# claforte/RayTracingWeekend.jl

Measured on AMD Instinct MI355X. Metric: Msamples/s (pixels x spp) on scene_random_spheres 1920x1080, higher is better.
Workload: dtype f32

## Files before the change

raytracingweekend.jl_amd/csrc/rtw_kernels.hpp:

```cpp
#pragma once
#include "rtw_device.hpp"

namespace rtw {

#define RTW_JOB_PX 16
#ifndef RTW_SLOT_BYTES
#define RTW_SLOT_BYTES 4608
#endif
#define RTW_REF_BITS 9
#define RTW_REF_MASK 511u
#define RTW_SLOT_FREE 0xffffffffu
#define RTW_SLOT_OPENING 0xfffffffeu
#define RTW_SLOT_OPENING_BIT 0x80000000u
#define RTW_JOB_EOF 0xffffffffu
#define RTW_JOB_RETRY 0xfffffffeu

struct KParams {
    int width, height, spp, max_depth;
    uint64_t seed;
    int n_chunks;
    int chunk_spp;
    int shard_index, shard_count;
    int tiles_i, tiles_j;
    unsigned total_jobs;
    unsigned local_tiles;
    unsigned bpj;
    unsigned n_slots, slot_stride;
    unsigned job_shift;
    unsigned rows_shift;
    unsigned div_bpj_m, div_bpj_s, div_tiles_m, div_tiles_s;
    int gamma;
    int out_layout;
    int drain_profile;
};

struct DevCounters {
    unsigned next_job[8];
    unsigned long long segments;
    unsigned long long samples;
    unsigned long long phase[32];
    unsigned long long t_first, t_last, t_end_sum, n_waves;
    unsigned end_hist[4096];
};

struct JobSlot {
    unsigned ready_seq;
    unsigned job;
    int remaining;
    unsigned valid;
    int i_base, j_base;
    unsigned k_tile;
    unsigned pad;
    double uv[12];
    __device__ __forceinline__ unsigned long long *acc(unsigned px) { return reinterpret_cast<unsigned long long *>(this + 1) + 8u * px; }
    __device__ __forceinline__ const unsigned long long *acc(unsigned px) const { return reinterpret_cast<const unsigned long long *>(this + 1) + 8u * px; }
};
static_assert(sizeof(JobSlot) == 128, "JobSlot header is 128 bytes (16-byte aligned accumulators follow)");
template <typename T> struct BatchArgs {
    const Camera<T> *cams;
    const unsigned long long *seeds;
    unsigned tiles_jv;
    unsigned div_tjv_m, div_tjv_s;
    unsigned long long view_elems;
};
struct AccumArgs {
    unsigned long long *words;
    int chunk_begin;
    int samples;
};
struct JobCache { unsigned long long jc; unsigned jc_lock; unsigned queue_off; unsigned last_g; unsigned static_used; };
template <typename T> struct WgShared {
    unsigned char slots[RTW_SLOT_BYTES];
    __device__ __forceinline__ JobSlot *slot(unsigned i, unsigned stride) { return reinterpret_cast<JobSlot *>(slots + i * stride); }
    unsigned ticket;
    unsigned eof;
    unsigned fin_waves;
    unsigned long long fin_segments, fin_samples;
    unsigned long long t_wave[8];
    JobCache jobs;
    Camera<T> cam;
    KParams P;
};

template <bool ON> struct PhaseClock {
    unsigned long long t0 = 0, acc[32] = {0, 0, 0, 0, 0, 0, 0, 0, 0, 0, 0, 0, 0, 0, 0, 0, 0, 0, 0, 0, 0, 0, 0, 0, 0, 0, 0, 0, 0, 0, 0, 0};
    __device__ __forceinline__ void start() { if (ON) t0 = __builtin_readcyclecounter(); }
    __device__ __forceinline__ void lap(int k) {
        if (ON) { unsigned long long t = __builtin_readcyclecounter(); acc[k] += t - t0; t0 = t; }
    }
    static constexpr bool on() { return ON; }
    __device__ __forceinline__ void count(int k, unsigned n) { if (ON) acc[k] += n; }
};

__device__ __forceinline__ unsigned udiv_magic(unsigned n, unsigned m, unsigned s) {
    if (s & 0x80000000u) return n;
    const unsigned t = __umulhi(n, m);
    return (t + ((n - t) >> 1)) >> s;
}

__device__ __forceinline__ unsigned lane_id() { return __builtin_amdgcn_mbcnt_hi(~0u, __builtin_amdgcn_mbcnt_lo(~0u, 0u)); }
__device__ __forceinline__ unsigned uniform(unsigned v) { return (unsigned)__builtin_amdgcn_readfirstlane((int)v); }

#ifndef RTW_TRACE_WAVES_F32
#define RTW_TRACE_WAVES_F32 7
#endif
#ifndef RTW_TRACE_WAVES_F64
#define RTW_TRACE_WAVES_F64 5
#endif
template <typename T> struct TraceWaves { static constexpr int value = RTW_TRACE_WAVES_F32; };
template <> struct TraceWaves<double> { static constexpr int value = RTW_TRACE_WAVES_F64; };
#ifndef RTW_TRACE_WAVES_CULL_F32
#define RTW_TRACE_WAVES_CULL_F32 5
#endif
template <typename T, bool CULL, bool MFMA = false> struct TraceWavesOf { static constexpr int value = TraceWaves<T>::value; };
template <> struct TraceWavesOf<float, true, false> { static constexpr int value = RTW_TRACE_WAVES_CULL_F32; };
template <> struct TraceWavesOf<double, true, false> { static constexpr int value = 3; };
#ifndef RTW_TRACE_WAVES_MFMA_F32
#define RTW_TRACE_WAVES_MFMA_F32 5
#endif
#ifndef RTW_TRACE_WAVES_MFMA_F64
#define RTW_TRACE_WAVES_MFMA_F64 4
#endif
template <> struct TraceWavesOf<float, false, true> { static constexpr int value = RTW_TRACE_WAVES_MFMA_F32; };
template <> struct TraceWavesOf<double, false, true> { static constexpr int value = RTW_TRACE_WAVES_MFMA_F64; };
template <> struct TraceWavesOf<float, true, true> { static constexpr int value = RTW_TRACE_WAVES_MFMA_F32; };
template <> struct TraceWavesOf<double, true, true> { static constexpr int value = RTW_TRACE_WAVES_MFMA_F64; };
template <typename T> __host__ __device__ constexpr size_t mfma_cell_bytes() { return 4 * (64 * sizeof(unsigned long long) + (sizeof(T) == 8 ? 64 * sizeof(unsigned) : 0)) + 4 * 64 * 16; }

#ifndef RTW_RARE_ATTR
#define RTW_RARE_ATTR __forceinline__
#endif

__device__ __forceinline__ void fx_accumulate(unsigned long long *a, double r, double g, double b) {
    const double cs[3] = {r, g, b};
#pragma unroll 1
    for (int c = 0; c < 3; ++c) {

        unsigned long long lo, hi;
        if (fx_from_double(cs[c], lo, hi)) {
            const unsigned long long old = __hip_atomic_fetch_add(&a[2 * c], lo, __ATOMIC_RELAXED, __HIP_MEMORY_SCOPE_WORKGROUP);
            hi += (old + lo < old) ? 1ull : 0ull;
            if (hi) __hip_atomic_fetch_add(&a[2 * c + 1], hi, __ATOMIC_RELAXED, __HIP_MEMORY_SCOPE_WORKGROUP);
        } else {
            __hip_atomic_fetch_add(&a[6], 1ull, __ATOMIC_RELAXED, __HIP_MEMORY_SCOPE_WORKGROUP);
        }
    }
}

__device__ __forceinline__ void fx_accumulate_channel(unsigned long long *acc, unsigned c, double v) {
    unsigned long long lo, hi;
    if (fx_from_double(v, lo, hi)) {
        const unsigned long long old = __hip_atomic_fetch_add(&acc[2 * c], lo, __ATOMIC_RELAXED, __HIP_MEMORY_SCOPE_WORKGROUP);
        hi += (old + lo < old) ? 1ull : 0ull;
        if (hi) __hip_atomic_fetch_add(&acc[2 * c + 1], hi, __ATOMIC_RELAXED, __HIP_MEMORY_SCOPE_WORKGROUP);
    } else {
        __hip_atomic_fetch_add(&acc[6], 1ull, __ATOMIC_RELAXED, __HIP_MEMORY_SCOPE_WORKGROUP);
    }
}

template <typename T>
__device__ RTW_RARE_ATTR void store_job(const KParams &P, const JobSlot *S, unsigned lane, T *__restrict__ out) {
    const unsigned px = lane / 3u, ch = lane - 3u * px, rs = P.rows_shift;
    if (px < (1u << P.job_shift)) {
        if ((S->valid >> px) & 1u) {
            const int i0 = S->i_base + (int)(px & ((1u << rs) - 1u)), j0 = S->j_base + (int)(px >> rs);
            const unsigned long long *a = S->acc(px);
            double v = fx_to_double(a[2 * ch], a[2 * ch + 1]);
            if (a[6] != 0ull) v = __builtin_nan("");
            v = v / (double)P.spp;
            if (P.gamma) v = __builtin_sqrt(v);
            const size_t pix = P.out_layout == 0 ? (size_t)j0 * (size_t)P.height + (size_t)i0
                                                 : (size_t)S->k_tile * 64u + (size_t)((i0 & 7) + 8 * (j0 & 7));
            out[pix * 3 + ch] = (T)v;
        }
    }
}

template <typename T>
__device__ RTW_RARE_ATTR void store_job_accum(const KParams &P, const JobSlot *S, unsigned lane, T *__restrict__ out, const AccumArgs &A) {
    const unsigned px = lane / 3u, ch = lane - 3u * px, rs = P.rows_shift;
    if (px < (1u << P.job_shift)) {
        if ((S->valid >> px) & 1u) {
            const int i0 = S->i_base + (int)(px & ((1u << rs) - 1u)), j0 = S->j_base + (int)(px >> rs);
            const size_t pix = (size_t)j0 * (size_t)P.height + (size_t)i0;
            const unsigned long long *a = S->acc(px);
            ulonglong2 *g = reinterpret_cast<ulonglong2 *>(A.words + pix * 8u);
            const unsigned long long poison = reinterpret_cast<const unsigned long long *>(g)[6] + a[6];
            const bool poisoned = poison != 0ull;
            if (ch == 0u) g[3] = ulonglong2{poison, 0ull};
            const ulonglong2 old = g[ch];
            const unsigned long long lo = old.x + a[2 * ch];
            const unsigned long long hi = old.y + a[2 * ch + 1] + (lo < old.x ? 1ull : 0ull);
            g[ch] = ulonglong2{lo, hi};
            if (out) {
                double v = fx_to_double(lo, hi);
                if (poisoned) v = __builtin_nan("");
                v = v / (double)A.samples;
                if (P.gamma) v = __builtin_sqrt(v);
                out[pix * 3 + ch] = (T)v;
            }
        }
    }
}

__device__ __forceinline__ unsigned xcd_id() { return (unsigned)__builtin_amdgcn_s_getreg((4 - 1) << 11 | 0 << 6 | 20) & 7u; }

__device__ __forceinline__ unsigned queue_tiles(const KParams &P, unsigned xq) {
    if (P.shard_count == 1) { const unsigned tj = (unsigned)P.tiles_j; return tj > xq ? ((tj - xq + 7u) >> 3) * (unsigned)P.tiles_i : 0u; }
    return P.local_tiles > xq ? (P.local_tiles - xq + 7u) >> 3 : 0u;
}
__device__ __forceinline__ unsigned queue_positions(const KParams &P, unsigned xq, unsigned sub_shift) { return queue_tiles(P, xq) << sub_shift; }

#ifndef RTW_JOB_CLAIM
#define RTW_JOB_CLAIM 8u
#endif
#ifndef RTW_CLAIM_TAIL
#define RTW_CLAIM_TAIL 16u
#endif
#ifndef RTW_OPEN_RETRY
#define RTW_OPEN_RETRY 1
#endif
#ifndef RTW_STATIC_CLAIMS
#define RTW_STATIC_CLAIMS 4u
#endif
__device__ __forceinline__ unsigned static_claims(unsigned xq, unsigned q_pos) {
    const unsigned wgs = (gridDim.x + 7u - xq) >> 3;
    const unsigned k = wgs ? q_pos / wgs : 0u;
    return k < RTW_STATIC_CLAIMS ? k : RTW_STATIC_CLAIMS;
}
__device__ __forceinline__ unsigned static_base(unsigned xq, unsigned q_pos) { return static_claims(xq, q_pos) * ((gridDim.x + 7u - xq) >> 3); }
__device__ __forceinline__ int claim_job(const KParams &P, DevCounters *ctr, JobCache *C, unsigned xcd, unsigned sub_shift, unsigned &xq_out, unsigned &gq_out) {
    constexpr unsigned long long M28 = (1ull << 28) - 1ull;
    if (__hip_atomic_load(&C->static_used, __ATOMIC_RELAXED, __HIP_MEMORY_SCOPE_WORKGROUP) < RTW_STATIC_CLAIMS) {
        const unsigned k = __hip_atomic_fetch_add(&C->static_used, 1u, __ATOMIC_RELAXED, __HIP_MEMORY_SCOPE_WORKGROUP);
        const unsigned xq = blockIdx.x & 7u, ks = static_claims(xq, queue_positions(P, xq, sub_shift));
        if (k < ks) { xq_out = xq; gq_out = (blockIdx.x >> 3) * ks + k; return 1; }
    }
    for (;;) {
        unsigned long long w = __hip_atomic_load(&C->jc, __ATOMIC_RELAXED, __HIP_MEMORY_SCOPE_WORKGROUP);
        while ((w & M28) < ((w >> 28) & M28)) {
            if (__hip_atomic_compare_exchange_strong(&C->jc, &w, w + 1ull, __ATOMIC_RELAXED, __ATOMIC_RELAXED, __HIP_MEMORY_SCOPE_WORKGROUP)) {
                xq_out = (unsigned)(w >> 56); gq_out = (unsigned)(w & M28);
                return 1;
            }
        }
        unsigned expect = 0u;
        const bool locked = __hip_atomic_compare_exchange_strong(&C->jc_lock, &expect, 1u, __ATOMIC_ACQUIRE, __ATOMIC_RELAXED, __HIP_MEMORY_SCOPE_WORKGROUP);
        if (locked) {
            w = __hip_atomic_load(&C->jc, __ATOMIC_RELAXED, __HIP_MEMORY_SCOPE_WORKGROUP);
            if ((w & M28) < ((w >> 28) & M28)) {
                __hip_atomic_store(&C->jc_lock, 0u, __ATOMIC_RELEASE, __HIP_MEMORY_SCOPE_WORKGROUP);
                continue;
            }
        }
        unsigned off = __hip_atomic_load(&C->queue_off, __ATOMIC_RELAXED, __HIP_MEMORY_SCOPE_WORKGROUP);
        bool got = false;
        while (off < 8u) {
            const unsigned xq = (xcd + off) & 7u;
            const unsigned q_pos = queue_positions(P, xq, sub_shift);
            const unsigned seen = __hip_atomic_load(&C->last_g, __ATOMIC_RELAXED, __HIP_MEMORY_SCOPE_WORKGROUP), left = q_pos > seen ? q_pos - seen : 0u;
            unsigned n = 1u;
            if (locked && off == 0u) { n = left / (RTW_CLAIM_TAIL * (gridDim.x / 8u + 1u)); n = n > RTW_JOB_CLAIM ? RTW_JOB_CLAIM : n < 1u ? 1u : n; }
            const unsigned g0 = atomicAdd(&ctr->next_job[xq], n) + static_base(xq, q_pos);
            if (off == 0u) __hip_atomic_store(&C->last_g, g0, __ATOMIC_RELAXED, __HIP_MEMORY_SCOPE_WORKGROUP);
            if (g0 >= q_pos) { off += 1u; continue; }
            xq_out = xq; gq_out = g0; got = true;
            const unsigned end = g0 + n < q_pos ? g0 + n : q_pos;
            if (locked && end > g0 + 1u)
                __hip_atomic_store(&C->jc, ((unsigned long long)xq << 56) | ((unsigned long long)end << 28) | (unsigned long long)(g0 + 1u), __ATOMIC_RELAXED, __HIP_MEMORY_SCOPE_WORKGROUP);
            break;
        }
        __hip_atomic_store(&C->queue_off, off, __ATOMIC_RELAXED, __HIP_MEMORY_SCOPE_WORKGROUP);
        if (locked) __hip_atomic_store(&C->jc_lock, 0u, __ATOMIC_RELEASE, __HIP_MEMORY_SCOPE_WORKGROUP);
        return got ? 1 : (locked ? 0 : 2);
    }
}

template <bool WITH_RETRY = false, bool BATCH = false>
__device__ RTW_RARE_ATTR void open_job(const KParams &P, JobSlot *S, unsigned lane, DevCounters *ctr, JobCache *jcache,
                                       unsigned tiles_jv = 0u, unsigned div_tjv_m = 0u, unsigned div_tjv_s = 0u) {
    unsigned g = RTW_JOB_EOF, valid = 0, k = 0;
    [[maybe_unused]] unsigned view = 0;
    int i_base = 0, j_base = 0;
    const unsigned rs = P.rows_shift, cs = P.job_shift - rs, sub_shift = 6u - P.job_shift, bps_shift = 3u - rs;
    const unsigned xcd = xcd_id();
    for (;;) {
        unsigned xq = 0, gq = 0, ok = 0;
        if (lane == 0) ok = (unsigned)claim_job(P, ctr, jcache, xcd, sub_shift, xq, gq);
        ok = uniform(ok);
        if (ok == 2u) { if (WITH_RETRY) { g = RTW_JOB_RETRY; break; } __builtin_amdgcn_s_sleep(1); continue; }
        if (!ok) break;
        xq = uniform(xq); gq = uniform(gq);
        const unsigned qt = gq >> sub_shift, q = gq & ((1u << sub_shift) - 1u);
        unsigned tj, ti;
        if (P.shard_count == 1) {
            const unsigned tjq = udiv_magic(qt, P.div_tiles_m, P.div_tiles_s);
            ti = qt - tjq * (unsigned)P.tiles_i; tj = xq + 8u * tjq;
            k = tj * (unsigned)P.tiles_i + ti;
            if constexpr (BATCH) { view = udiv_magic(tj, div_tjv_m, div_tjv_s); tj -= view * tiles_jv; }
        } else {
            k = xq + 8u * qt;
            const unsigned t = k * (unsigned)P.shard_count + (unsigned)P.shard_index;
            tj = udiv_magic(t, P.div_tiles_m, P.div_tiles_s); ti = t - tj * (unsigned)P.tiles_i;
        }
        i_base = (int)(ti * 8u + ((q & ((1u << bps_shift) - 1u)) << rs));
        j_base = (int)(tj * 8u + ((q >> bps_shift) << cs));
        const int i0 = i_base + (int)(lane & ((1u << rs) - 1u)), j0 = j_base + (int)((lane >> rs) & ((1u << cs) - 1u));
        valid = (unsigned)__ballot(lane < (1u << P.job_shift) && i0 < P.height && j0 < P.width);
        if (valid) { g = gq; break; }
    }
    if (g < RTW_JOB_RETRY) {
        if (lane < (4u << P.job_shift)) {
            unsigned zero = 0u;
            __asm__ volatile("" : "+v"(zero));
            reinterpret_cast<uint4 *>(S->acc(0))[lane] = uint4{zero, zero, zero, zero};
        }
        if (lane < 4) S->uv[lane] = (double)(j_base + (int)lane + 1) / (double)P.width;
        else if (lane < 12) S->uv[lane] = (double)(P.height - (i_base + (int)lane - 4 + 1)) / (double)P.height;
        if (lane == 0) {
            S->remaining = (int)((unsigned)__popc(valid) * (unsigned)P.n_chunks);
            S->valid = valid; S->i_base = i_base; S->j_base = j_base; S->k_tile = k;
            if constexpr (BATCH) S->pad = view;
        }
    }
    if (lane == 0) S->job = g;
}

template <typename T, bool PROFILE, bool LDS_SCENE, bool CULL, bool MFMA = false, int NUMK = -1, bool BATCH = false, bool ACCUM = false>
__global__ __launch_bounds__(256, (TraceWavesOf<T, CULL, MFMA>::value)) void trace_kernel(KParams P_arg, Camera<T> cam_arg, DevScene<T> scene,
                                                   CullScene<T> cull, T *__restrict__ out, DevCounters *ctr, BatchArgs<T> batch, AccumArgs accum) {
    static_assert(!(BATCH && ACCUM) && !(PROFILE && ACCUM), "no batched and no phase-profile ACCUM instances");
    using V4 = typename Vec4<T>::type;
    if constexpr (NUMK >= 0) { scene.numerics = NUMK; cull.numerics = NUMK; }
    const unsigned lane = lane_id();
    extern __shared__ __attribute__((aligned(16))) unsigned char smem[];
    unsigned short *my_list = reinterpret_cast<unsigned short *>(smem) + threadIdx.x;
    constexpr size_t list_bytes = RTW_LIST_CAP * 256 * sizeof(unsigned short);
    constexpr size_t shared_bytes = (sizeof(WgShared<T>) + 15) / 16 * 16;
    WgShared<T> *sh = reinterpret_cast<WgShared<T> *>(smem + list_bytes);
    constexpr size_t cell_bytes = MFMA ? mfma_cell_bytes<T>() : 0;
    V4 *lds_geom = reinterpret_cast<V4 *>(smem + list_bytes + shared_bytes + cell_bytes);
    WaveScratch ws = {nullptr, nullptr, nullptr};
    [[maybe_unused]] ulonglong2 *pool_rng = nullptr;
    [[maybe_unused]] unsigned long long pool_valid = 0;
    if constexpr (MFMA) {
        static_assert(list_bytes == 4 * RTW_PAIR_CAP * sizeof(unsigned), "the pair lists reuse the per-lane list area");
        const unsigned wv = threadIdx.x >> 6;
        unsigned char *cells = smem + list_bytes + shared_bytes;
        ws.pairs = reinterpret_cast<unsigned *>(smem) + wv * RTW_PAIR_CAP;
        ws.keys = reinterpret_cast<unsigned long long *>(cells) + wv * 64;
        ws.kidx = reinterpret_cast<unsigned *>(cells + 4 * 64 * sizeof(unsigned long long)) + wv * 64;
        pool_rng = reinterpret_cast<ulonglong2 *>(cells + mfma_cell_bytes<T>() - 4 * 64 * 16) + wv * 64;
    }
    unsigned short *lds_orig = reinterpret_cast<unsigned short *>(lds_geom + (CULL ? cull_exact_count(cull) : 0));
    [[maybe_unused]] unsigned *lds_tab = reinterpret_cast<unsigned *>(reinterpret_cast<unsigned char *>(lds_orig) + (CULL ? ((size_t)cull_exact_count(cull) * sizeof(unsigned short) + 15) / 16 * 16 : 0));
    if (threadIdx.x < P_arg.n_slots) { JobSlot *S0 = sh->slot(threadIdx.x, P_arg.slot_stride); S0->ready_seq = RTW_SLOT_FREE; S0->job = 0u; }
    if (threadIdx.x == 0) { sh->ticket = 0u; sh->eof = 0u; sh->fin_waves = 0u; sh->fin_segments = 0ull; sh->fin_samples = 0ull; sh->jobs.jc = 0ull; sh->jobs.jc_lock = 0u; sh->jobs.queue_off = 0u; sh->jobs.last_g = 0u; sh->jobs.static_used = 0u; sh->cam = cam_arg; sh->P = P_arg; }
    const KParams &P = sh->P;
    if (LDS_SCENE) {
        if (CULL) stage_cull_scene<T>(cull, lds_geom, lds_orig);
        else stage_scene<T>(scene, lds_geom);
        if constexpr (CULL && MFMA) {
            const unsigned *gt = reinterpret_cast<const unsigned *>(cull.mf_box + 8 * (cull.mf_blocks + 1));
            for (int i = threadIdx.x; i < cull_tab_words(cull.mf_blocks); i += blockDim.x) lds_tab[i] = gt[i];
        }
    }
    __syncthreads();

    if (lane == 0 && (threadIdx.x >> 6) < 4u) sh->t_wave[threadIdx.x >> 6] = wall_clock64();
    unsigned pool_next = 0, pool_end = 0;
    unsigned pool_slot = 0, pool_b = 0;
    bool have_ticket = false;
    unsigned tk_seq = 0, tk_b = 0;

    unsigned long long n_segments = 0, n_samples = 0;

    bool alive = true;
    bool have_item = false;
    bool has_ray = false;
    unsigned ref_depth = 0;
    int samples_left = 0;
    bool jitter = false;
    Rng rng = {1, 2};
    V3<T> ro = {0, 0, 0}, rd = {0, 0, 1};
    double thr_r = 1, thr_g = 1, thr_b = 1;
    const T w_div = (T)(float)P.width;
    const T h_div = (T)(float)P.height;

    PhaseClock<PROFILE> clk;
    for (;;) {
        clk.start();
        T t_hit = 0;
        int idx = -1;
        if constexpr (MFMA && CULL) {
            if (__any(has_ray)) {
                MfmaCull mc = mfma_cull_of(cull);
                if (LDS_SCENE) mc.tab = lds_tab;
                if (LDS_SCENE) idx = hit_world_mfma<T>(scene, (const V4 *)lds_geom, ro, rd, has_ray, (T)1e-4, t_hit, ws, lane, clk, &mc, (const unsigned short *)lds_orig);
                else idx = hit_world_mfma<T>(scene, cull.exact, ro, rd, has_ray, (T)1e-4, t_hit, ws, lane, clk, &mc, cull.orig);
            }
        } else if constexpr (MFMA) {
            if (__any(has_ray)) {
                if (LDS_SCENE) idx = hit_world_mfma<T>(scene, (const V4 *)lds_geom, ro, rd, has_ray, (T)1e-4, t_hit, ws, lane, clk);
                else idx = hit_world_mfma<T>(scene, scene.geom, ro, rd, has_ray, (T)1e-4, t_hit, ws, lane, clk);
            }
        } else if (has_ray) {
            if (CULL && LDS_SCENE)
                idx = hit_world_cull<T, 256>(cull, (const V4 *)lds_geom, (const unsigned short *)lds_orig, ro, rd, (T)1e-4,
                                             (T)__builtin_huge_val(), t_hit, my_list, clk);
            else if (CULL)
                idx = hit_world_cull<T, 256>(cull, cull.exact, cull.orig, ro, rd, (T)1e-4, (T)__builtin_huge_val(), t_hit, my_list, clk);
            else if (LDS_SCENE)
                idx = hit_world<T, 256>(scene, (const V4 *)lds_geom, ro, rd, (T)1e-4, (T)__builtin_huge_val(), t_hit, my_list, clk);
            else
                idx = hit_world<T, 256>(scene, scene.geom, ro, rd, (T)1e-4, (T)__builtin_huge_val(), t_hit, my_list, clk);
        }
        n_segments += (unsigned long long)__popcll(__ballot(has_ray));
        clk.lap(2);
        if (PROFILE) { clk.count(8, 1u); clk.count(9, (unsigned)__popcll(__ballot(has_ray))); if (!__any(has_ray)) clk.count(10, 1u); }

        const bool hit = has_ray && idx >= 0;
        if constexpr (MFMA) {
            const bool miss = RTW_PROBE_MISS(has_ray && idx < 0);
            const unsigned long long miss_mask = __ballot(miss);
            if (miss_mask) {
                clk.count(18, 1u); clk.count(19, (3u * (unsigned)__popcll(miss_mask) + 63u) / 64u);
                unsigned char *scr = reinterpret_cast<unsigned char *>(ws.pairs);
                double *task_val = reinterpret_cast<double *>(scr);
                unsigned short *task_acc = reinterpret_cast<unsigned short *>(scr + 1536);
                if (miss) {
                    const C3 sky = skycolor(rd);
                    const unsigned k3 = 3u * __builtin_amdgcn_mbcnt_hi((unsigned)(miss_mask >> 32), __builtin_amdgcn_mbcnt_lo((unsigned)miss_mask, 0u));
                    const unsigned item_ref = ref_depth & RTW_REF_MASK;
                    const unsigned a0 = (unsigned)(reinterpret_cast<unsigned char *>(sh->slot(item_ref >> 4, P.slot_stride)->acc(item_ref & 15u)) - smem);
                    task_val[k3] = thr_r * sky.r; task_val[k3 + 1u] = thr_g * sky.g; task_val[k3 + 2u] = thr_b * sky.b;
                    task_acc[k3] = (unsigned short)a0; task_acc[k3 + 1u] = (unsigned short)(a0 | 1u); task_acc[k3 + 2u] = (unsigned short)(a0 | 2u);
                }
                __builtin_amdgcn_wave_barrier();
                const unsigned n3 = 3u * (unsigned)__popcll(miss_mask);
                for (unsigned t0 = 0; t0 < n3; t0 += 64u) {
                    const unsigned t = t0 + lane;
                    if (t < n3) {
                        const unsigned ac = task_acc[t];
                        fx_accumulate_channel(reinterpret_cast<unsigned long long *>(smem + (ac & 0xfff8u)), ac & 7u, task_val[t]);
                    }
                }
                __builtin_amdgcn_wave_barrier();
            }
        } else if (has_ray && idx < 0) {
            const C3 sky = skycolor(rd);
            const unsigned item_ref = ref_depth & RTW_REF_MASK;
            fx_accumulate(sh->slot(item_ref >> 4, P.slot_stride)->acc(item_ref & 15u), thr_r * sky.r, thr_g * sky.g, thr_b * sky.b);
        }
        has_ray = false;

        const bool need = alive && !hit && samples_left == 0;
        const unsigned long long need_mask = __ballot(need);
        if (need_mask) {
            clk.count(20, 1u);
            bool last = false;
            if (need && have_item) {
                last = __hip_atomic_fetch_add(&sh->slot((ref_depth & RTW_REF_MASK) >> 4, P.slot_stride)->remaining, -1, __ATOMIC_ACQ_REL, __HIP_MEMORY_SCOPE_WORKGROUP) == 1;
                have_item = false;
            }
            unsigned long long fin = __ballot(last);
            while (fin) {
                const int L = __builtin_ctzll(fin);
                fin &= fin - 1ull;
                JobSlot *S = sh->slot(uniform((unsigned)__shfl((int)((ref_depth & RTW_REF_MASK) >> 4), L)), P.slot_stride);
                if constexpr (BATCH) store_job<T>(P, S, lane, out + (size_t)uniform(S->pad) * batch.view_elems);
                else if constexpr (ACCUM) store_job_accum<T>(P, S, lane, out, accum);
                else store_job<T>(P, S, lane, out);
                clk.count(21, 1u);
                __hip_atomic_store(&S->ready_seq, RTW_SLOT_FREE, __ATOMIC_RELEASE, __HIP_MEMORY_SCOPE_WORKGROUP);
            }
#pragma unroll 1
            for (int round = 0; round < 2; ++round) {
                const bool taker = need && alive && !have_item;
                const unsigned long long take_mask = __ballot(taker);
                if (!take_mask) break;
                if (pool_next >= pool_end) {
                    if (!have_ticket) {
                        unsigned t = 0;
                        if (lane == 0) t = __hip_atomic_fetch_add(&sh->ticket, 1u, __ATOMIC_RELAXED, __HIP_MEMORY_SCOPE_WORKGROUP);
                        t = uniform(t);
                        tk_seq = udiv_magic(t, P.div_bpj_m, P.div_bpj_s);
                        tk_b = t - tk_seq * P.bpj;
                        have_ticket = true;
                    }
                    const unsigned eof = uniform(__hip_atomic_load(&sh->eof, __ATOMIC_ACQUIRE, __HIP_MEMORY_SCOPE_WORKGROUP));
                    unsigned rs = RTW_SLOT_OPENING;
                    if (lane < P.n_slots) rs = __hip_atomic_load(&sh->slot(lane, P.slot_stride)->ready_seq, __ATOMIC_ACQUIRE, __HIP_MEMORY_SCOPE_WORKGROUP);
                    unsigned long long m_mine = __ballot(rs == tk_seq);
                    const unsigned long long m_opening = __ballot(rs == (tk_seq | RTW_SLOT_OPENING_BIT)), m_free = __ballot(rs == RTW_SLOT_FREE);
                    unsigned sl = 0;
                    if (!m_mine && !m_opening && !eof && tk_b == 0u && m_free) {
                        sl = (unsigned)__builtin_ctzll(m_free);
                        JobSlot *S = sh->slot(sl, P.slot_stride);
                        unsigned won = 0;
                        if (lane == 0) {
                            unsigned expect = RTW_SLOT_FREE;
                            won = __hip_atomic_compare_exchange_strong(&S->ready_seq, &expect, tk_seq | RTW_SLOT_OPENING_BIT, __ATOMIC_ACQ_REL,
                                                                       __ATOMIC_RELAXED, __HIP_MEMORY_SCOPE_WORKGROUP) ? 1u : 0u;
                        }
                        if (uniform(won)) {
                            if constexpr (BATCH) open_job<RTW_OPEN_RETRY != 0, true>(P, S, lane, ctr, &sh->jobs, batch.tiles_jv, batch.div_tjv_m, batch.div_tjv_s);
                            else open_job<RTW_OPEN_RETRY != 0>(P, S, lane, ctr, &sh->jobs);
                            const unsigned opened = uniform(S->job);
                            if (opened >= RTW_JOB_RETRY) {
                                if (opened == RTW_JOB_EOF && lane == 0) __hip_atomic_store(&sh->eof, 1u, __ATOMIC_RELEASE, __HIP_MEMORY_SCOPE_WORKGROUP);
                                __hip_atomic_store(&S->ready_seq, RTW_SLOT_FREE, __ATOMIC_RELEASE, __HIP_MEMORY_SCOPE_WORKGROUP);
                                if (opened == RTW_JOB_EOF) {
                                    if (taker) alive = false;
                                    have_ticket = false;
                                }
                                break;
                            }
                            __hip_atomic_store(&S->ready_seq, tk_seq, __ATOMIC_RELEASE, __HIP_MEMORY_SCOPE_WORKGROUP);
                            m_mine = 1ull << sl;
                        }
                    } else if (!m_mine && !m_opening && eof) {
                        if (taker) alive = false;
                        have_ticket = false;
                        break;
                    }
                    if (!m_mine) break;
                    sl = (unsigned)__builtin_ctzll(m_mine);
                    const JobSlot *S = sh->slot(sl, P.slot_stride);
                    clk.count(22, 1u);
                    pool_slot = sl; pool_b = tk_b;
                    pool_next = 0; pool_end = 64;
                    have_ticket = false;
                    if constexpr (MFMA) {
                        const unsigned px = lane & ((1u << P.job_shift) - 1u), chunk = tk_b * (64u >> P.job_shift) + (lane >> P.job_shift);
                        const unsigned rsh = P.rows_shift;
                        const int i0 = S->i_base + (int)(px & ((1u << rsh) - 1u)), j0 = S->j_base + (int)(px >> rsh);
                        Rng r0;
                        if constexpr (BATCH) rng_stream(batch.seeds[uniform(S->pad)], (unsigned long long)j0 * (unsigned)P.height + (unsigned)i0, chunk, r0);
                        else if constexpr (ACCUM) rng_stream(P.seed, (unsigned long long)j0 * (unsigned)P.height + (unsigned)i0, chunk + (unsigned)accum.chunk_begin, r0);
                        else rng_stream(P.seed, (unsigned long long)j0 * (unsigned)P.height + (unsigned)i0, chunk, r0);
                        __builtin_amdgcn_wave_barrier();
                        pool_rng[lane] = ulonglong2{r0.x, r0.y};
                        pool_valid = __ballot((int)chunk < P.n_chunks && ((S->valid >> px) & 1u));
                        __builtin_amdgcn_wave_barrier();
                    }
                }
                const unsigned rank = __builtin_amdgcn_mbcnt_hi((unsigned)(take_mask >> 32), __builtin_amdgcn_mbcnt_lo((unsigned)take_mask, 0u));
                const unsigned p = pool_next + rank;
                if (taker && p < pool_end) {
                    const JobSlot *S = sh->slot(pool_slot, P.slot_stride);
                    const unsigned px = p & ((1u << P.job_shift) - 1u), chunk = pool_b * (64u >> P.job_shift) + (p >> P.job_shift);
                    bool real;
                    if constexpr (MFMA) real = ((pool_valid >> p) & 1ull) != 0ull;
                    else real = (int)chunk < P.n_chunks && ((S->valid >> px) & 1u);
                    if (real) {
                        if constexpr (MFMA) {
                            const ulonglong2 st = pool_rng[p];
                            rng.x = st.x; rng.y = st.y;
                        } else {
                            const unsigned rsh = P.rows_shift;
                            const int i0 = S->i_base + (int)(px & ((1u << rsh) - 1u)), j0 = S->j_base + (int)(px >> rsh);
                            const unsigned long long pix = (unsigned long long)j0 * (unsigned)P.height + (unsigned)i0;
                            if constexpr (BATCH) rng_stream(batch.seeds[uniform(S->pad)], pix, chunk, rng);
                            else if constexpr (ACCUM) rng_stream(P.seed, pix, chunk + (unsigned)accum.chunk_begin, rng);
                            else rng_stream(P.seed, pix, chunk, rng);
                        }
                        int s0 = (int)chunk * P.chunk_spp;
                        if constexpr (ACCUM) s0 = (int)(chunk + (unsigned)accum.chunk_begin) * P.chunk_spp;
                        samples_left = min(P.spp, s0 + P.chunk_spp) - s0;
                        jitter = s0 != 0;
                        ref_depth = pool_slot * 16u + px;
                        have_item = true;
                    }
                }
                const unsigned want = (unsigned)__popcll(take_mask), have = pool_end - pool_next;
                if (PROFILE && want > have) clk.count(11, want - have);
                pool_next = min(pool_end, pool_next + want);
                if (want <= have) break;
            }
            if (PROFILE) clk.count(12, (unsigned)__popcll(__ballot(need && alive && !have_item)));
        }
        if (!__any(alive)) break;
        clk.lap(0);

        int todo = PATH_READY;
        V3<T> vec = {0, 0, 0};
        T vscale_ = 1;
        int kind = 0;
        if (PROFILE && __any(hit)) clk.count(23, 1u);
        if (hit) {
            const V4 g = CULL ? cull.exact[idx] : scene.geom[idx];
            const V4 m0 = CULL ? cull.mat0[idx] : scene.mat0[idx];
            const V4 m1 = CULL ? cull.mat1[idx] : scene.mat1[idx];
            HitRec<T> rec;
            make_hitrec<T>({g.x, g.y, g.z}, m0.x, ro, rd, t_hit, rec);
            kind = (int)m0.z;
            const DielConst<T> dc = {m0.w, m1.x, m1.y};
            todo = scatter_begin<T>(rng, kind, m0.y, rd, rec, vec, vscale_, &dc);
            const V3<T> att = attenuation_of<T>(kind, {m1.x, m1.y, m1.z});
            thr_r = thr_r * (double)att.x; thr_g = thr_g * (double)att.y; thr_b = thr_b * (double)att.z;
            ro = rec.p;
            ref_depth -= 1u << RTW_REF_BITS;
            if (todo == PATH_READY) { rd = vec; has_ray = ref_depth > RTW_REF_MASK; }
        }
        clk.lap(3);

        bool new_sample = false;
        T su = 0, sv = 0;
        if (alive && !hit && samples_left > 0) {
            T du = 0, dv = 0;
            if (jitter) {
                T r1, r2;
                trand(rng, r1); du = RTW_DIV(r1, w_div);
                trand(rng, r2); dv = RTW_DIV(r2, h_div);
            }
            const JobSlot *S = sh->slot((ref_depth & RTW_REF_MASK) >> 4, P.slot_stride);
            const unsigned px = ref_depth & 15u;
            const unsigned rs = P.rows_shift;
            su = (T)S->uv[px >> rs] + du;
            sv = (T)S->uv[4 + (px & ((1u << rs) - 1u))] + dv;
            new_sample = true;
            jitter = true;
            samples_left -= 1;
        }
        n_samples += (unsigned long long)__popcll(__ballot(new_sample));
        if (PROFILE && __any(new_sample)) clk.count(24, 1u);

        const bool ball = todo == PATH_BALL;
        V3<T> rp = {0, 0, 0};
        T len2 = 0;
        {
            bool pending = ball || new_sample;
            RTW_PROBE_REJECT_TWICE();
            constexpr bool use_prio = MFMA && sizeof(T) == 4 && RTW_SCAN_PRIO != 0;
            if (use_prio) __builtin_amdgcn_s_setprio(0);
#ifdef RTW_PROBE_REJ_CAP
            for (int rr = 0; rr < RTW_PROBE_REJ_CAP && pending; ++rr) {
                len2 = reject_trial<T>(rng, ball, rp);
                pending = !(len2 <= T(1));
            }
            if (pending) len2 = T(1);
#else
            if constexpr (PROFILE) {
                if (__any(pending)) clk.count(17, 1u);
                while (__any(pending)) {
                    clk.count(16, 1u);
                    if (__any(ball && pending)) clk.count(29, 1u);
                    if (pending) { len2 = reject_trial<T>(rng, ball, rp); pending = !(len2 <= T(1)); }
                }
            }
            while (pending) {
                len2 = reject_trial<T>(rng, ball, rp);
                pending = !(len2 <= T(1));
            }
#endif
            if (use_prio) __builtin_amdgcn_s_setprio(1);
        }
        if (ball) {
            todo = scatter_finish<T>(kind, vec, vscale_, rp, len2, vec);
            if (todo == PATH_READY) rd = vec;
        }
        if (new_sample) {
            __asm__ volatile("" ::: "memory");
            if constexpr (BATCH) {
                const Camera<T> cam = batch.cams[sh->slot((ref_depth & RTW_REF_MASK) >> 4, P.slot_stride)->pad];
                camera_ray_raw<T>(cam, su, sv, rp.x, rp.y, ro, vec);
            } else {
                const Camera<T> cam = sh->cam;
                camera_ray_raw<T>(cam, su, sv, rp.x, rp.y, ro, vec);
            }
            todo = PATH_NORM;
            thr_r = thr_g = thr_b = 1.0;
            ref_depth = (ref_depth & RTW_REF_MASK) | ((unsigned)P.max_depth << RTW_REF_BITS);
        }
        if (PROFILE && __any(todo == PATH_NORM)) clk.count(25, 1u);
        if (todo == PATH_NORM) rd = normalize(vec);
        if (ball || new_sample || todo == PATH_NORM) has_ray = ref_depth > RTW_REF_MASK;
        clk.lap(1);
        if (!__any(has_ray)) __builtin_amdgcn_s_sleep(2);
    }

    if (PROFILE && lane == 0) {
        for (int k = 0; k < 32; ++k) atomicAdd(&ctr->phase[k], clk.acc[k]);
    }
    if (lane == 0) {
        __hip_atomic_fetch_add(&sh->fin_segments, n_segments, __ATOMIC_RELAXED, __HIP_MEMORY_SCOPE_WORKGROUP);
        __hip_atomic_fetch_add(&sh->fin_samples, n_samples, __ATOMIC_RELAXED, __HIP_MEMORY_SCOPE_WORKGROUP);
        if ((threadIdx.x >> 6) < 4u) __hip_atomic_store(&sh->t_wave[4u + (threadIdx.x >> 6)], wall_clock64(), __ATOMIC_RELAXED, __HIP_MEMORY_SCOPE_WORKGROUP);
        const unsigned nw = blockDim.x >> 6;
        if (__hip_atomic_fetch_add(&sh->fin_waves, 1u, __ATOMIC_ACQ_REL, __HIP_MEMORY_SCOPE_WORKGROUP) == nw - 1u) {
            atomicAdd(&ctr->segments, __hip_atomic_load(&sh->fin_segments, __ATOMIC_RELAXED, __HIP_MEMORY_SCOPE_WORKGROUP));
            atomicAdd(&ctr->samples, __hip_atomic_load(&sh->fin_samples, __ATOMIC_RELAXED, __HIP_MEMORY_SCOPE_WORKGROUP));
            if (P.drain_profile) {
            unsigned long long t_start = ~0ull, t_end = 0ull, t_sum = 0ull;
            for (unsigned w = 0; w < nw && w < 4u; ++w) {
                const unsigned long long a = __hip_atomic_load(&sh->t_wave[w], __ATOMIC_RELAXED, __HIP_MEMORY_SCOPE_WORKGROUP);
                const unsigned long long e = __hip_atomic_load(&sh->t_wave[4u + w], __ATOMIC_RELAXED, __HIP_MEMORY_SCOPE_WORKGROUP);
                t_start = a < t_start ? a : t_start; t_end = e > t_end ? e : t_end; t_sum += e;
            }
            const unsigned long long t0_seen = atomicMin(&ctr->t_first, t_start);
            atomicMax(&ctr->t_last, t_end);
            atomicAdd(&ctr->t_end_sum, t_sum);
            atomicAdd(&ctr->n_waves, (unsigned long long)nw);
            const unsigned long long t0 = t0_seen < t_start ? t0_seen : t_start;
            for (unsigned w = 0; w < nw && w < 4u; ++w) {
                const unsigned long long bin = (__hip_atomic_load(&sh->t_wave[4u + w], __ATOMIC_RELAXED, __HIP_MEMORY_SCOPE_WORKGROUP) - t0) / 25000ull;
                atomicAdd(&ctr->end_hist[bin < 4095ull ? (unsigned)bin : 4095u], 1u);
            }
            }
        }
    }
}

}
```

raytracingweekend.jl_amd/csrc/rtw_path.hpp:

```cpp
#pragma once
#include <hip/hip_runtime.h>
#include <stdint.h>

namespace rtw {


enum { LAMBERTIAN = 0, METAL = 1, DIELECTRIC = 2 };

template <typename T> struct V3 { T x, y, z; };
struct C3 { double r, g, b; };

template <typename T> struct Vec4;
template <> struct Vec4<float> { using type = float4; };
template <> struct Vec4<double> { using type = double4; };

#ifndef RTW_EXACT_FAST_MATH
#define RTW_EXACT_FAST_MATH 1
#endif
__device__ __forceinline__ float t_sqrt(float x) {
#if RTW_EXACT_FAST_MATH
    if (__all(x >= 0x1p-100f && x <= 0x1p100f)) {
        const float y = __builtin_amdgcn_rsqf(x);
        float g = x * y, h = 0.5f * y;
        const float r = __builtin_fmaf(-h, g, 0.5f);
        g = __builtin_fmaf(g, r, g); h = __builtin_fmaf(h, r, h);
        const float d = __builtin_fmaf(-g, g, x);
        return __builtin_fmaf(d, h, g);
    }
#endif
    return __builtin_sqrtf(x);
}
__device__ __forceinline__ double t_sqrt(double x) { return __builtin_sqrt(x); }
__device__ __forceinline__ float t_rcp(float x) {
#if RTW_EXACT_FAST_MATH
    if (__all(__builtin_fabsf(x) >= 0x1p-100f && __builtin_fabsf(x) <= 0x1p100f)) {
        float y = __builtin_amdgcn_rcpf(x);
        float e = __builtin_fmaf(-x, y, 1.0f);
        y = __builtin_fmaf(e, y, y);
        e = __builtin_fmaf(-x, y, 1.0f);
        return __builtin_fmaf(e, y, y);
    }
#endif
    return 1.0f / x;
}
__device__ __forceinline__ double t_rcp(double x) { return 1.0 / x; }
__device__ __forceinline__ float t_fma(float a, float b, float c) { return __builtin_fmaf(a, b, c); }
__device__ __forceinline__ double t_fma(double a, double b, double c) { return __builtin_fma(a, b, c); }

template <typename T> __device__ __forceinline__ V3<T> vadd(V3<T> a, V3<T> b) { return {a.x + b.x, a.y + b.y, a.z + b.z}; }
template <typename T> __device__ __forceinline__ V3<T> vsub(V3<T> a, V3<T> b) { return {a.x - b.x, a.y - b.y, a.z - b.z}; }
template <typename T> __device__ __forceinline__ V3<T> vscale(T s, V3<T> a) { return {s * a.x, s * a.y, s * a.z}; }
template <typename T> __device__ __forceinline__ V3<T> vneg(V3<T> a) { return {-a.x, -a.y, -a.z}; }
template <typename T> __device__ __forceinline__ T dot(V3<T> a, V3<T> b) { return (a.x * b.x + a.y * b.y) + a.z * b.z; }
#include "rtw_probes.hpp"
#ifdef RTW_PROBE_FASTDIV
__device__ __forceinline__ float probe_rsq(float x) { return __builtin_amdgcn_rsqf(x); }
__device__ __forceinline__ double probe_rsq(double x) { return 1.0 / __builtin_sqrt(x); }
__device__ __forceinline__ float probe_rcp(float x) { return __builtin_amdgcn_rcpf(x); }
__device__ __forceinline__ double probe_rcp(double x) { return 1.0 / x; }
#endif
template <typename T> __device__ __forceinline__ V3<T> normalize(V3<T> a) {
    T inv = RTW_RSQRT(dot(a, a));
    return vscale(inv, a);
}
template <typename T> __device__ __forceinline__ bool near_zero(V3<T> a) { return (double)dot(a, a) < 1e-5; }

struct Rng { uint64_t x, y; };

__device__ __forceinline__ uint32_t funnel(uint32_t hi, uint32_t lo, uint32_t s) { return __builtin_amdgcn_alignbit(hi, lo, s); }
__device__ __forceinline__ uint64_t rng_next(Rng &r) {
    const uint32_t xl = (uint32_t)r.x, xh = (uint32_t)(r.x >> 32), yl = (uint32_t)r.y, yh = (uint32_t)(r.y >> 32);
    const uint64_t out = r.x + r.y;
    const uint32_t sl = xl ^ yl, sh = xh ^ yh;
    const uint32_t nxl = __builtin_amdgcn_bitop3_b32(funnel(xh, xl, 9), sl, sl << 14, 0x96);
    const uint32_t nxh = __builtin_amdgcn_bitop3_b32(funnel(xl, xh, 9), sh, funnel(sh, sl, 18), 0x96);
    r.x = ((uint64_t)nxh << 32) | nxl;
    r.y = ((uint64_t)funnel(sl, sh, 28) << 32) | funnel(sh, sl, 28);
    return out;
}
__device__ __forceinline__ uint64_t splitmix64(uint64_t &s) {
    uint64_t z = (s += 0x9e3779b97f4a7c15ULL);
    z = (z ^ (z >> 30)) * 0xbf58476d1ce4e5b9ULL;
    z = (z ^ (z >> 27)) * 0x94d049bb133111ebULL;
    return z ^ (z >> 31);
}
__device__ __forceinline__ void rng_stream(uint64_t seed, uint64_t pixel, uint64_t chunk, Rng &r) {
    uint64_t p1 = pixel + 1, c1 = chunk + 1;
    __asm__ volatile("" : "+v"(p1), "+v"(c1));
    uint64_t s = seed ^ (0xd1b54a32d192ed03ULL * p1) ^ (0x8cb92ba72f3d8dd7ULL * c1);
    r.x = splitmix64(s);
    r.y = splitmix64(s);
    (void)rng_next(r);
}
__device__ __forceinline__ void trand(Rng &r, float &out) {
    uint32_t bits = ((uint32_t)rng_next(r) & 0x007fffffu) | 0x3f800000u;
    __asm__("v_add_f32_e32 %0, -1.0, %1" : "=v"(out) : "v"(__uint_as_float(bits)));
}
__device__ __forceinline__ void trand(Rng &r, double &out) {
    uint64_t bits = (rng_next(r) & 0x000fffffffffffffULL) | 0x3ff0000000000000ULL;
    out = __longlong_as_double((long long)bits) - 1.0;
}
template <typename T> __device__ __forceinline__ T random_between(Rng &r, T mn, T mx) {
    T u; trand(r, u);
    return u * (mx - mn) + mn;
}
__device__ __forceinline__ float random_pm1(Rng &r, float) {
    const uint32_t bits = ((uint32_t)rng_next(r) & 0x007fffffu) | 0x3f800000u;
    return __builtin_fmaf(__uint_as_float(bits), 2.0f, -3.0f);
}
__device__ __forceinline__ double random_pm1(Rng &r, double) {
    const uint64_t bits = (rng_next(r) & 0x000fffffffffffffULL) | 0x3ff0000000000000ULL;
    return __builtin_fma(__longlong_as_double((long long)bits), 2.0, -3.0);
}
template <typename T> __device__ __forceinline__ T reject_trial(Rng &r, bool ball, V3<T> &p) {
    p.x = random_pm1(r, T(0));
    p.y = random_pm1(r, T(0));
    p.z = T(0);
    if (ball) p.z = random_pm1(r, T(0));
    return (p.x * p.x + p.y * p.y) + p.z * p.z;
}
template <typename T> __device__ __forceinline__ V3<T> normalize_len2(V3<T> p, T len2) {
    return vscale(RTW_RSQRT(len2), p);
}
template <typename T> __device__ __forceinline__ V3<T> random_vec3_on_sphere(Rng &r) {
    V3<T> p; T len2;
    do { len2 = reject_trial<T>(r, true, p); } while (!(len2 <= T(1)));
    return normalize_len2(p, len2);
}
template <typename T> __device__ __forceinline__ void random_vec2_in_disk(Rng &r, T &x, T &y) {
    V3<T> p; T len2;
    do { len2 = reject_trial<T>(r, false, p); } while (!(len2 <= T(1)));
    x = p.x; y = p.y;
}

enum { NUM_REFERENCE = 0, NUM_CONTRACT = 1, NUM_REFERENCE_FMA2 = 3 };
template <int N> struct NumTag { static constexpr int value = N; };
template <typename T, int NUM>
__device__ __forceinline__ void sphere_disc_n(T cx, T cy, T cz, T r2, [[maybe_unused]] T r, V3<T> o, V3<T> d, T &half_b, T &disc) {
    const T ocx = o.x - cx, ocy = o.y - cy, ocz = o.z - cz;
    if constexpr (NUM == NUM_CONTRACT) {
        half_b = t_fma(ocz, d.z, t_fma(ocy, d.y, ocx * d.x));
        const T nc = t_fma(-ocz, ocz, t_fma(-ocy, ocy, t_fma(-ocx, ocx, r2)));
        disc = t_fma(half_b, half_b, nc);
    } else {
        half_b = (ocx * d.x + ocy * d.y) + ocz * d.z;
        const T ococ = (ocx * ocx + ocy * ocy) + ocz * ocz;
        const T c = (NUM == NUM_REFERENCE_FMA2 && !(r2 < T(0))) ? t_fma(-r, r, ococ) : ococ - r2;
        if constexpr (NUM == NUM_REFERENCE) disc = half_b * half_b - c;
        else disc = t_fma(half_b, half_b, -c);
    }
}
template <typename T>
__device__ __forceinline__ void sphere_disc(int num, T cx, T cy, T cz, T r2, T r, V3<T> o, V3<T> d, T &half_b, T &disc) {
    if (num == NUM_REFERENCE) sphere_disc_n<T, NUM_REFERENCE>(cx, cy, cz, r2, r, o, d, half_b, disc);
    else if (num == NUM_CONTRACT) sphere_disc_n<T, NUM_CONTRACT>(cx, cy, cz, r2, r, o, d, half_b, disc);
    else sphere_disc_n<T, NUM_REFERENCE_FMA2>(cx, cy, cz, r2, r, o, d, half_b, disc);
}
template <typename T>
__device__ __forceinline__ bool sphere_root(T half_b, T disc, T tmin, T closest, T &root) {
    if (disc < T(0)) return false;
    T sqrtd = t_sqrt(disc);
    root = -half_b - sqrtd;
    if (root < tmin || closest < root) {
        root = -half_b + sqrtd;
        if (root < tmin || closest < root) return false;
    }
    return true;
}

template <typename T> struct HitRec { T t; V3<T> p, n; bool front; };

template <typename T>
__device__ __forceinline__ void make_hitrec(V3<T> c, T r, V3<T> o, V3<T> d, T t, HitRec<T> &rec) {
    rec.t = t;
    rec.p = vadd(o, vscale(t, d));
    V3<T> pc = vsub(rec.p, c);
    V3<T> n_out = {RTW_DIV(pc.x, r), RTW_DIV(pc.y, r), RTW_DIV(pc.z, r)};
    rec.front = dot(d, n_out) < T(0);
    rec.n = rec.front ? n_out : vneg(n_out);
}

template <typename T> __device__ __forceinline__ V3<T> reflect(V3<T> v, V3<T> n) {
    T k = dot(vscale(T(2), v), n);
    return vsub(v, vscale(k, n));
}
template <typename T> __device__ __forceinline__ V3<T> refract_raw(V3<T> dir, V3<T> n, T ratio) {
    T cos_t = -dot(dir, n);
    if (!(T(1) > cos_t)) cos_t = T(1);
    V3<T> perp = vscale(ratio, vadd(dir, vscale(cos_t, n)));
    T one_m = T(1) - dot(perp, perp);
    T par_s = -t_sqrt(one_m < T(0) ? -one_m : one_m);
    return vadd(perp, vscale(par_s, n));
}
template <typename T> __device__ __forceinline__ V3<T> refract(V3<T> dir, V3<T> n, T ratio) {
    return normalize(refract_raw(dir, n, ratio));
}
template <typename T> __device__ __forceinline__ T reflectance(T cos_t, T ratio) {
    T r0 = (T(1) - ratio) / (T(1) + ratio);
    r0 = r0 * r0;
    T x = T(1) - cos_t;
    T x2 = x * x;
    T x5 = (x2 * x2) * x;
    return r0 + (T(1) - r0) * x5;
}

enum { PATH_READY = 0,
       PATH_NORM = 1,
       PATH_BALL = 2 };
template <typename T> struct DielConst { T inv_ir, r0_front, r0_back; };
template <typename T> __host__ __device__ inline DielConst<T> dielectric_constants(T ir) {
    DielConst<T> c;
    c.inv_ir = T(1) / ir;
    T a = (T(1) - c.inv_ir) / (T(1) + c.inv_ir); c.r0_front = a * a;
    T b = (T(1) - ir) / (T(1) + ir); c.r0_back = b * b;
    return c;
}
template <typename T> __device__ __forceinline__ T reflectance_r0(T cos_t, T r0) {
    T x = T(1) - cos_t;
    T x2 = x * x;
    T x5 = (x2 * x2) * x;
    return r0 + (T(1) - r0) * x5;
}
template <typename T>
__device__ __forceinline__ int scatter_begin(Rng &rng, int kind, T param, V3<T> d_in, const HitRec<T> &rec,
                                             V3<T> &vec, T &scale, const DielConst<T> *dc = nullptr) {
    scale = T(1);
    if (kind == DIELECTRIC) {
        T ratio = dc ? (rec.front ? dc->inv_ir : param) : (rec.front ? (T(1) / param) : param);
        T cos_t = -dot(d_in, rec.n);
        if (!(T(1) > cos_t)) cos_t = T(1);
        T sin_t = t_sqrt(T(1) - cos_t * cos_t);
        bool refl = ratio * sin_t > T(1);
        if (!refl) {
            T u; trand(rng, u);
            refl = (dc ? reflectance_r0(cos_t, rec.front ? dc->r0_front : dc->r0_back) : reflectance(cos_t, ratio)) > u;
        }
        if (refl) { vec = reflect(d_in, rec.n); return PATH_READY; }
        vec = refract_raw(d_in, rec.n, ratio);
        return PATH_NORM;
    }
    if (kind == LAMBERTIAN) { vec = rec.n; } else { vec = reflect(d_in, rec.n); scale = param; }
    return PATH_BALL;
}
template <typename T>
__device__ __forceinline__ int scatter_finish(int kind, V3<T> base, T scale, V3<T> p, T len2, V3<T> &vec) {
    V3<T> uvec = normalize_len2(p, len2);
    V3<T> dir = vadd(base, vscale(scale, uvec));
    if (kind == LAMBERTIAN && near_zero(dir)) { vec = base; return PATH_READY; }
    vec = dir;
    return PATH_NORM;
}
template <typename T> __device__ __forceinline__ V3<T> attenuation_of(int kind, V3<T> albedo) {
    return kind == DIELECTRIC ? V3<T>{T(1), T(1), T(1)} : albedo;
}
template <typename T>
__device__ __forceinline__ void scatter(Rng &rng, int kind, V3<T> albedo, T param, V3<T> d_in,
                                        const HitRec<T> &rec, V3<T> &out_d, V3<T> &att) {
    att = attenuation_of(kind, albedo);
    V3<T> vec; T scale;
    int path = scatter_begin<T>(rng, kind, param, d_in, rec, vec, scale);
    if (path == PATH_BALL) {
        V3<T> p; T len2;
        do { len2 = reject_trial<T>(rng, true, p); } while (!(len2 <= T(1)));
        path = scatter_finish<T>(kind, vec, scale, p, len2, vec);
    }
    out_d = path == PATH_NORM ? normalize(vec) : vec;
}

template <typename T> __device__ __forceinline__ C3 skycolor(V3<T> d) {
    T t = T(0.5) * (d.y + T(1));
    T omt = T(1) - t;
    return {(double)omt * 1.0 + (double)t * 0.5, (double)omt * 1.0 + (double)t * 0.7,
            (double)omt * 1.0 + (double)t * 1.0};
}

template <typename T> struct Camera {
    T origin[3], llc[3], horizontal[3], vertical[3], u[3], v[3], w[3];
    T lens_radius;
};
template <typename T>
__device__ __forceinline__ void camera_ray_raw(const Camera<T> &cam, T s, T t, T dx, T dy, V3<T> &ro, V3<T> &raw) {
    T rx = cam.lens_radius * dx, ry = cam.lens_radius * dy;
    V3<T> cu = {cam.u[0], cam.u[1], cam.u[2]}, cv = {cam.v[0], cam.v[1], cam.v[2]};
    V3<T> org = {cam.origin[0], cam.origin[1], cam.origin[2]};
    V3<T> llc = {cam.llc[0], cam.llc[1], cam.llc[2]};
    V3<T> hor = {cam.horizontal[0], cam.horizontal[1], cam.horizontal[2]};
    V3<T> ver = {cam.vertical[0], cam.vertical[1], cam.vertical[2]};
    V3<T> offset = vadd(vscale(rx, cu), vscale(ry, cv));
    ro = vadd(org, offset);
    V3<T> dir = vadd(llc, vscale(s, hor));
    dir = vadd(dir, vscale(t, ver));
    dir = vsub(dir, org);
    raw = vsub(dir, offset);
}
template <typename T>
__device__ __forceinline__ void get_ray(Rng &rng, const Camera<T> &cam, T s, T t, V3<T> &ro, V3<T> &rd) {
    T dx, dy;
    random_vec2_in_disk(rng, dx, dy);
    V3<T> raw;
    camera_ray_raw(cam, s, t, dx, dy, ro, raw);
    rd = normalize(raw);
}

__device__ __forceinline__ bool fx_from_double(double x, unsigned long long &lo, unsigned long long &hi) {
    const double a = __builtin_fabs(x);
    if (!(a < 2147483648.0)) return false;
    const unsigned ip = (unsigned)a;
    const double fr = a - (double)ip;
    const double y = fr * 4294967296.0;
    const unsigned p1 = (unsigned)y;
    const double r1 = y - (double)p1;
    const unsigned p0 = (unsigned)(r1 * 4294967296.0);
    unsigned long long l = ((unsigned long long)p1 << 32) | (unsigned long long)p0, h = ip;
    if (x < 0.0) { l = 0ull - l; h = ~h + (l == 0ull ? 1ull : 0ull); }
    lo = l; hi = h;
    return true;
}
__device__ __forceinline__ double fx_to_double(unsigned long long lo, unsigned long long hi) {
    const bool neg = (long long)hi < 0;
    if (neg) { lo = 0ull - lo; hi = ~hi + (lo == 0ull ? 1ull : 0ull); }
    if ((lo | hi) == 0ull) return 0.0;
    const int n = hi ? __clzll((long long)hi) : 64 + __clzll((long long)lo);
    if (n >= 64) { hi = lo << (n - 64); lo = 0ull; }
    else if (n > 0) { hi = (hi << n) | (lo >> (64 - n)); lo <<= n; }
    unsigned long long mant = hi >> 11;
    const unsigned rem = (unsigned)hi & 0x7ffu;
    const bool sticky = lo != 0ull;
    if (rem > 0x400u || (rem == 0x400u && (sticky || (mant & 1ull)))) mant += 1ull;
    const double v = __builtin_ldexp((double)mant, 11 - n);
    return neg ? -v : v;
}

}
```

raytracingweekend.jl_amd/csrc/rtw_probes.hpp:

```cpp
#pragma once

#ifdef RTW_DUP_OPERANDS
#define RTW_PROBE_OPERANDS_TWICE()                                                                                                          \
    {                                                                                                                                       \
        float ox2 = ox, oy2 = oy, oz2 = oz, dx2_ = dx, dy2_ = dy, dz2_ = dz;                                                                \
        __asm__ volatile("" : "+v"(ox2), "+v"(oy2), "+v"(oz2), "+v"(dx2_), "+v"(dy2_), "+v"(dz2_));                                         \
        const float q_ = __builtin_fmaf(oz2, dz2_, __builtin_fmaf(oy2, dy2_, ox2 * dx2_));                                                  \
        const float oo_ = __builtin_fmaf(oz2, oz2, __builtin_fmaf(oy2, oy2, ox2 * ox2));                                                    \
        const float o1_ = (__builtin_fabsf(ox2) + __builtin_fabsf(oy2)) + __builtin_fabsf(oz2);                                             \
        const float oop_ = __builtin_fmaf(oo_, w.mf_oo_keep, -(w.mf_o1_coef * o1_));                                                        \
        const float tq_ = w.mf_sigma2 * __builtin_fmaf(q_, q_, -oop_);                                                                      \
        const float fp_[3] = {__builtin_fmaf(-q_, dx2_, ox2) * zs2, __builtin_fmaf(-q_, dy2_, oy2) * zs2, __builtin_fmaf(-q_, dz2_, oz2) * zs2}; \
        const float ax_ = dx2_ * z2, ay_ = dy2_ * z2, az_ = dz2_ * z2;                                                                      \
        const float fq_[6] = {ax_ * dx2_, ay_ * dy2_, az_ * dz2_, (ax_ + ax_) * dy2_, (ax_ + ax_) * dz2_, (ay_ + ay_) * dz2_};              \
        unsigned sq_[6], sp_[3];                                                                                                            \
        for (int k = 0; k < 6; ++k) sq_[k] = split_f16(fq_[k]);                                                                             \
        for (int k = 0; k < 3; ++k) sp_[k] = split_f16(fp_[k]);                                                                             \
        const float tx_ = ok ? tq_ : tx;                                                                                                    \
        const _Float16 t1_ = (_Float16)(tx_ * (1.0f / 32768.0f));                                                                           \
        const unsigned x23_ = split_f16((tx_ - 32768.0f * (float)t1_) * (1.0f / 16.0f));                                                    \
        const unsigned a0[8] = {dup(sq_[0]), cat(sq_[0], sq_[1]), sq_[1], dup(sq_[2]), sq_[5], dup(sp_[0]), cat(sp_[0], sp_[1]), sp_[1]};   \
        const unsigned a1[8] = {cat(sq_[2], sq_[3]), sq_[3], dup(sq_[4]), cat(sq_[4], sq_[5]), dup(sp_[2]), cat(sp_[2], sb),                \
                                ss | ((unsigned)__builtin_bit_cast(unsigned short, t1_) << 16), x23_};                                      \
        for (int k = 0; k < 8; ++k) {                                                                                                       \
            const auto sw2 = __builtin_amdgcn_permlane32_swap(a0[k], a1[k], false, false);                                                  \
            __asm__ volatile("" :: "v"(sw2[0]), "v"(sw2[1]));                                                                               \
        }                                                                                                                                   \
    }
#else
#define RTW_PROBE_OPERANDS_TWICE()
#endif

#ifdef RTW_PROBE_NO_MFMA
#define RTW_PROBE_FILTER_PAIR_REPLACED(a1, a2, b1, b2)                                                                                      \
    {                                                                                                                                       \
        rtw_f16v Wn = {-1, -1, -1, -1, -1, -1, -1, -1, -1, -1, -1, -1, -1, -1, -1, -1};                                                     \
        const uint4 u1 = __builtin_bit_cast(uint4, b1), u2 = __builtin_bit_cast(uint4, b2);                                                 \
        __asm__ volatile("" :: "v"(a1.x), "v"(a1.y), "v"(a1.z), "v"(a1.w), "v"(a2.x), "v"(a2.y), "v"(a2.z), "v"(a2.w));                     \
        __asm__ volatile("" :: "v"(u1.x), "v"(u1.y), "v"(u1.z), "v"(u1.w), "v"(u2.x), "v"(u2.y), "v"(u2.z), "v"(u2.w));                     \
        __asm__ volatile("" : "+v"(Wn));                                                                                                    \
        return Wn;                                                                                                                          \
    }
#else
#define RTW_PROBE_FILTER_PAIR_REPLACED(a1, a2, b1, b2)
#endif

#ifdef RTW_DUP_MFMA
#define RTW_PROBE_FILTER_PAIR_AGAIN(Wp, a1, a2, b1, b2)                                                                                     \
    for (int rep = 0; rep < (RTW_DUP_MFMA + 0 > 0 ? RTW_DUP_MFMA + 0 : 1); ++rep) {                                                         \
        uint4 a1c = a1;                                                                                                                     \
        __asm__ volatile("" : "+v"(a1c.x), "+v"(a1c.y), "+v"(a1c.z), "+v"(a1c.w));                                                          \
        __asm__ volatile("" : "+v"(Wp));                                                                                                    \
        Wp = __builtin_amdgcn_mfma_f32_32x32x16_f16(__builtin_bit_cast(rtw_h8, a1c), b1, zero, 0, 0, 0);                                    \
        Wp = __builtin_amdgcn_mfma_f32_32x32x16_f16(__builtin_bit_cast(rtw_h8, a2), b2, Wp, 0, 0, 0);                                       \
    }
#else
#define RTW_PROBE_FILTER_PAIR_AGAIN(Wp, a1, a2, b1, b2)
#endif

#ifdef RTW_DUP_EVAL
#define RTW_PROBE_EVAL_TWICE(Wv) { unsigned keep = mask; eval(Wv); __asm__ volatile("" :: "v"(mask)); mask = keep; __asm__ volatile("" : "+v"(Wv)); }
#else
#define RTW_PROBE_EVAL_TWICE(Wv)
#endif

#ifdef RTW_DUP_EXTRACT
#define RTW_PROBE_EXTRACT_TWICE()                                                                                                           \
    {                                                                                                                                       \
        unsigned m2 = m; __asm__ volatile("" : "+v"(m2));                                                                                   \
        const unsigned long long act2 = __ballot(m2 != 0u);                                                                                 \
        if (m2 != 0u) reinterpret_cast<uint2 *>(ws.pairs)[__builtin_amdgcn_mbcnt_hi((unsigned)(act2 >> 32), __builtin_amdgcn_mbcnt_lo((unsigned)act2, total))] = uint2{m2, lane_const + (unsigned)cur * 32u}; \
        __builtin_amdgcn_wave_barrier();                                                                                                    \
    }
#else
#define RTW_PROBE_EXTRACT_TWICE()
#endif

#ifdef RTW_DUP_RESOLVE_PAIRS
#define RTW_PROBE_RESOLVE_TWICE() resolve_pairs<T>(w.numerics, src, rad, o, d, tmin, ws, total, lane, orig)
#else
#define RTW_PROBE_RESOLVE_TWICE()
#endif

#ifdef RTW_DUP_REJECT
#define RTW_PROBE_REJECT_TWICE()                                                                                                            \
    {                                                                                                                                       \
        Rng r2 = rng; V3<T> q2 = {0, 0, 0}; T l2 = 0; bool p2 = pending;                                                                    \
        while (__any(p2)) { if (p2) { l2 = reject_trial<T>(r2, ball, q2); p2 = !(l2 <= T(1)); } }                                           \
        __asm__ volatile("" :: "v"(q2.x), "v"(q2.y), "v"(q2.z), "v"(l2), "v"((unsigned)r2.x), "v"((unsigned)r2.y));                         \
    }
#else
#define RTW_PROBE_REJECT_TWICE()
#endif

#ifdef RTW_PROBE_NO_ACCUM
#define RTW_PROBE_MISS(expr) false
#else
#define RTW_PROBE_MISS(expr) (expr)
#endif

#ifdef RTW_PROBE_FASTDIV
#define RTW_DIV(a, b) ((a) * ::rtw::probe_rcp(b))
#define RTW_RSQRT(x) ::rtw::probe_rsq(x)
#else
#define RTW_DIV(a, b) ((a) / (b))
#define RTW_RSQRT(x) t_rcp(t_sqrt(x))
#endif
```

raytracingweekend.jl_amd/csrc/rtw_scan.hpp:

```cpp
#pragma once
#include "rtw_path.hpp"

namespace rtw {

#define RTW_SPHERE_WORD 32
#define RTW_SPHERE_TAIL 8
__host__ __device__ inline int scene_geom_alloc(int n, int n_pad) {
    const int a = n_pad + RTW_SPHERE_TAIL, b = ((n + 31) / 32) * 32;
    return a > b ? a : b;
}
template <typename T> struct DevScene {
    const float *scan;
    const typename Vec4<T>::type *geom;
    const typename Vec4<T>::type *mat0;
    const typename Vec4<T>::type *mat1;
    int n, n_pad;
    const uint4 *mf_ops;
    int mf_blocks;
    float mf_sc;
    float mf_sigma2;
    float mf_oo_keep;
    float mf_o1_coef;
    float mf_o_max;
    int n_huge, huge[2];
    int numerics;
};

#define RTW_LIST_CAP 16
#define RTW_LDS_SCENE_MAX_BYTES (24 * 1024)

__device__ __forceinline__ uint32_t sign_word(float x) { return __float_as_uint(x); }
__device__ __forceinline__ uint32_t sign_word(double x) { return (uint32_t)((uint64_t)__double_as_longlong(x) >> 32); }

#ifndef RTW_SCAN_PRIO
#define RTW_SCAN_PRIO 1
#endif
template <typename T> struct ScanGroup;
template <> struct ScanGroup<float> { static constexpr int N = 4; };
template <> struct ScanGroup<double> { static constexpr int N = 4; };

struct NoClock { static constexpr bool on() { return false; } __device__ __forceinline__ void lap(int) {} __device__ __forceinline__ void count(int, unsigned) {} };
struct NoSink {
    static constexpr bool on() { return false; }
    unsigned self = 0;
    __device__ __forceinline__ void ray(unsigned, bool, float) {}
    __device__ __forceinline__ void cand(unsigned, int) {}
    __device__ __forceinline__ void inlane(unsigned, int) {}
};

template <typename T, int STRIDE, int NUM, typename SRC>
__device__ __forceinline__ void resolve_candidates_n(SRC src, const typename Vec4<T>::type *rad, V3<T> o, V3<T> d, T tmin, T &closest, int &idx,
                                                     const unsigned short *list, int cnt) {
    using V4 = typename Vec4<T>::type;
    auto test = [&](int c, int i, const V4 &s) {
        if (c < cnt) {
            T hb, disc, root, r = T(0);
            if constexpr (NUM == NUM_REFERENCE_FMA2) r = rad[i].x;
            sphere_disc_n<T, NUM>(s.x, s.y, s.z, s.w, r, o, d, hb, disc);
            if (sphere_root<T>(hb, disc, tmin, closest, root)) { closest = root; idx = i; }
        }
    };
    int ia = cnt > 0 ? (int)list[0] : 0;
    V4 sa = src[ia];
    for (int c = 0; __any(c < cnt); c += 2) {
        const int ib = (c + 1 < cnt) ? (int)list[(c + 1) * STRIDE] : 0;
        const V4 sb = src[ib];
        test(c, ia, sa);
        ia = (c + 2 < cnt) ? (int)list[(c + 2) * STRIDE] : 0;
        sa = src[ia];
        if (__any(c + 1 < cnt)) test(c + 1, ib, sb);
    }
}
template <typename T, int STRIDE, typename SRC>
__device__ __forceinline__ void resolve_candidates(int num, SRC src, const typename Vec4<T>::type *rad, V3<T> o, V3<T> d, T tmin, T &closest, int &idx,
                                                   const unsigned short *list, int cnt) {
    if (num == NUM_REFERENCE) resolve_candidates_n<T, STRIDE, NUM_REFERENCE>(src, rad, o, d, tmin, closest, idx, list, cnt);
    else if (num == NUM_CONTRACT) resolve_candidates_n<T, STRIDE, NUM_CONTRACT>(src, rad, o, d, tmin, closest, idx, list, cnt);
    else resolve_candidates_n<T, STRIDE, NUM_REFERENCE_FMA2>(src, rad, o, d, tmin, closest, idx, list, cnt);
}

template <typename T, int STRIDE, typename SRC, typename CLK = NoClock, typename SINK = NoSink>
__device__ __forceinline__ int hit_world(const DevScene<T> &w, SRC src, V3<T> o, V3<T> d, T tmin, T tmax, T &t_hit,
                                         unsigned short *list, CLK &&clk = NoClock(), SINK sink = SINK()) {
    constexpr int G = ScanGroup<T>::N;
    constexpr bool F64 = sizeof(T) == 8;
    constexpr int SW = F64 ? 8 : 4;
    typedef const float __attribute__((address_space(4))) *cptr;
    cptr gs = (cptr)(uintptr_t)w.scan;
    struct Unit { float v[SW]; };
    auto ldg = [&](int i) -> Unit {
        Unit r;
#pragma unroll
        for (int j = 0; j < SW; ++j) r.v[j] = gs[SW * i + j];
        return r;
    };
    T closest = tmax;
    int idx = -1, cnt = 0;
    Unit A[G], B[G];
#pragma unroll
    for (int k = 0; k < G; ++k) A[k] = ldg(k);
    [[maybe_unused]] bool lane_ok = true;
    [[maybe_unused]] V3<float> of = {0, 0, 0}, df = {0, 0, 1};
    if constexpr (F64) {
        const double s2 = dot(d, d), o2 = dot(o, o);
        lane_ok = s2 <= 1.001 && o2 < 1e30;
        of = {(float)o.x, (float)o.y, (float)o.z};
        df = {(float)d.x, (float)d.y, (float)d.z};
    }
    if constexpr (SINK::on()) sink.ray(sink.self, lane_ok, 0.0f);
    auto test1 = [&](auto tag, const Unit &sp, uint32_t &mask) {
        if constexpr (F64) {
            const float ocx = of.x - sp.v[0], ocy = of.y - sp.v[1], ocz = of.z - sp.v[2];
            const float hb = __builtin_fmaf(ocz, df.z, __builtin_fmaf(ocy, df.y, ocx * df.x));
            const float nc = __builtin_fmaf(-ocz, ocz, __builtin_fmaf(-ocy, ocy, __builtin_fmaf(-ocx, ocx, sp.v[3])));
            const float m = __builtin_fmaf(nc, 0.999996185302734375f , sp.v[4]);
            const float W = __builtin_fmaf(hb, hb, m);
            mask = __builtin_amdgcn_alignbit(mask, __float_as_uint(W), 31);
        } else {
            T hb, disc;
            if constexpr (decltype(tag)::value == NUM_REFERENCE_FMA2) {
                const T ocx = o.x - sp.v[0], ocy = o.y - sp.v[1], ocz = o.z - sp.v[2];
                hb = (ocx * d.x + ocy * d.y) + ocz * d.z;
                const T ococ = (ocx * ocx + ocy * ocy) + ocz * ocz;
                disc = t_fma(ococ + sp.v[3], T(4.76837158203125e-07), t_fma(hb, hb, -(ococ - sp.v[3])));
            } else {
                sphere_disc_n<T, decltype(tag)::value>(sp.v[0], sp.v[1], sp.v[2], sp.v[3], T(0), o, d, hb, disc);
            }
            if constexpr (decltype(tag)::value == NUM_CONTRACT) {
                const uint32_t u = sign_word(disc);
                mask = __builtin_amdgcn_alignbit(mask, u - (u >> 31), 31);
            } else {
                mask = __builtin_amdgcn_alignbit(mask, sign_word(disc), 31);
            }
        }
    };
    auto scan = [&](auto tag) {
    for (int base = 0; base < w.n_pad; base += RTW_SPHERE_WORD) {
        uint32_t mask = 0;
        const int left = w.n_pad - base;
        const int ngroups = (left >= RTW_SPHERE_WORD ? RTW_SPHERE_WORD : left) / G;
        const int npairs = ngroups >> 1;
        for (int q = 0; q < npairs; ++q) {
            const int off = base + q * 2 * G;
            test1(tag, A[0], mask);
            __builtin_amdgcn_sched_barrier(0);
#pragma unroll
            for (int k = 0; k < G; ++k) B[k] = ldg(off + G + k);
            __builtin_amdgcn_sched_barrier(0);
#pragma unroll
            for (int k = 1; k < G; ++k) test1(tag, A[k], mask);
            __builtin_amdgcn_sched_barrier(0);
            test1(tag, B[0], mask);
            __builtin_amdgcn_sched_barrier(0);
#pragma unroll
            for (int k = 0; k < G; ++k) A[k] = ldg(off + 2 * G + k);
            __builtin_amdgcn_sched_barrier(0);
#pragma unroll
            for (int k = 1; k < G; ++k) test1(tag, B[k], mask);
            __builtin_amdgcn_sched_barrier(0);
        }
        if (ngroups & 1) {
#pragma unroll
            for (int k = 0; k < G; ++k) test1(tag, A[k], mask);
        }
        clk.lap(2);
        uint32_t m = ~mask;
        if constexpr (F64) { if (!lane_ok) m = 0xffffffffu; }
        if (left < RTW_SPHERE_WORD) m <<= (RTW_SPHERE_WORD - ngroups * G);
        if constexpr (SINK::on()) for (uint32_t s_ = m; s_ != 0u; s_ &= s_ - 1u) sink.cand(sink.self, base + 31 - (int)__builtin_ctz(s_));
        auto push_first = [&]() {
            const int b = __clz((int)m);
            list[cnt * STRIDE] = (unsigned short)(base + b);
            cnt += 1;
            m &= ~(0x80000000u >> b);
        };
        if (!__any(m != 0u)) {
        } else if (!__any(cnt + (int)__popc(m) > RTW_LIST_CAP)) {
            do { if (m != 0u) push_first(); } while (__any(m != 0u));
        } else {
            while (__any(m != 0u)) {
                if (__any(cnt >= RTW_LIST_CAP)) {
                    clk.lap(4);
                    resolve_candidates<T, STRIDE>(w.numerics, src, w.mat0, o, d, tmin, closest, idx, list, cnt);
                    cnt = 0;
                    clk.lap(5);
                }
                if (m != 0u) push_first();
            }
        }
        clk.lap(4);
    }
    };
    if constexpr (F64) scan(NumTag<NUM_REFERENCE>{});
    else if (w.numerics == NUM_REFERENCE) scan(NumTag<NUM_REFERENCE>{});
    else if (w.numerics == NUM_CONTRACT) scan(NumTag<NUM_CONTRACT>{});
    else scan(NumTag<NUM_REFERENCE_FMA2>{});
    resolve_candidates<T, STRIDE>(w.numerics, src, w.mat0, o, d, tmin, closest, idx, list, cnt);
    clk.lap(5);
    t_hit = closest;
    return idx;
}

}
```

raytracingweekend.jl_amd/csrc/rtw_scan_cull.hpp:

```cpp
#pragma once
#include "rtw_scan_mfma.hpp"

namespace rtw {

#ifndef RTW_CULL_GS
#define RTW_CULL_GS 16
#endif
#define RTW_CULL_BG 4
#ifndef RTW_CULL_L2
#define RTW_CULL_L2 4
#endif
template <typename T> struct CullScene {
    const T *box;
    const typename Vec4<T>::type *exact;
    const unsigned short *orig;
    const typename Vec4<T>::type *mat0;
    const typename Vec4<T>::type *mat1;
    int n_groups_pad;
    int n_big;
    T cs[3], rs;
    T kappa;
    const uint4 *mf_ops;
    const float *mf_box;
    float mf_glo[3], mf_ghi[3];
    int mf_blocks;
    int n_huge, n_huge_exact;
    CullGrid grid;
    int numerics;
};
template <typename T> __host__ __device__ inline MfmaCull mfma_cull_of(const CullScene<T> &c) {
    return MfmaCull{c.mf_ops, c.mf_box, c.mf_blocks, {(float)c.cs[0], (float)c.cs[1], (float)c.cs[2]}, (float)c.rs * 1.000001f + 1e-30f, (const void *)c.mat0,
                    {c.mf_glo[0], c.mf_glo[1], c.mf_glo[2]}, {c.mf_ghi[0], c.mf_ghi[1], c.mf_ghi[2]}, c.n_huge, c.n_huge_exact, c.grid, reinterpret_cast<const unsigned *>(c.mf_box + 8 * (c.mf_blocks + 1))};
}
template <typename T> __host__ __device__ inline int cull_exact_count(const CullScene<T> &c) { return c.n_groups_pad * RTW_CULL_GS + ((c.n_big + 31) / 32) * 32; }

__device__ __forceinline__ float t_min(float a, float b) { return __builtin_fminf(a, b); }
__device__ __forceinline__ float t_max(float a, float b) { return __builtin_fmaxf(a, b); }
__device__ __forceinline__ double t_min(double a, double b) { return __builtin_fmin(a, b); }
__device__ __forceinline__ double t_max(double a, double b) { return __builtin_fmax(a, b); }

template <typename T, int STRIDE, typename SRC, typename ORIG>
__device__ __forceinline__ void resolve_candidates_anyorder(int num, SRC src, const typename Vec4<T>::type *rad, ORIG orig, V3<T> o, V3<T> d, T tmin, T &closest, int &idx,
                                                            const unsigned short *list, int cnt) {
    using V4 = typename Vec4<T>::type;
    int i_next = cnt > 0 ? (int)list[0] : 0;
    V4 s_next = src[i_next];
    for (int c = 0; __any(c < cnt); ++c) {
        const int i = i_next;
        const V4 s = s_next;
        i_next = (c + 1 < cnt) ? (int)list[(c + 1) * STRIDE] : 0;
        s_next = src[i_next];
        if (c < cnt) {
            T hb, disc, root;
            T rr = T(0);
            if (num == NUM_REFERENCE_FMA2) rr = rad[i].x;
            sphere_disc<T>(num, s.x, s.y, s.z, s.w, rr, o, d, hb, disc);
            if (sphere_root<T>(hb, disc, tmin, closest, root)) {
                bool take = true;
                if (root == closest && idx >= 0) take = orig[i] > orig[idx];
                if (take) { closest = root; idx = i; }
            }
        }
    }
}

template <typename T, int STRIDE, typename SRC, typename ORIG, typename CLK = NoClock, typename SINK = NoSink>
__device__ __forceinline__ int hit_world_cull(const CullScene<T> &w, SRC src, ORIG orig, V3<T> o, V3<T> d, T tmin, T tmax,
                                              T &t_hit, unsigned short *list, CLK &&clk = NoClock(), SINK sink = SINK()) {
    using V4 = typename Vec4<T>::type;
    constexpr int G = RTW_CULL_BG;
    constexpr int GS = RTW_CULL_GS;
    typedef const T __attribute__((address_space(4))) *cptr;
    cptr gx = (cptr)(uintptr_t)w.exact;
    T closest = tmax;
    int idx = -1, cnt = 0;
    auto push = [&](int i) {
        if (cnt >= RTW_LIST_CAP) {
            resolve_candidates_anyorder<T, STRIDE>(w.numerics, src, w.mat0, orig, o, d, tmin, closest, idx, list, cnt);
            cnt = 0;
        }
        list[cnt * STRIDE] = (unsigned short)i;
        cnt += 1;
        if constexpr (SINK::on()) sink.cand(sink.self, (int)orig[i]);
    };
    if constexpr (SINK::on()) sink.ray(sink.self, true, 0.0f);
    auto member = [&](const V4 &sp, int i) {
        T hb, disc;
        T rr = T(0);
        if (w.numerics == NUM_REFERENCE_FMA2) rr = w.mat0[i].x;
        sphere_disc<T>(w.numerics, sp.x, sp.y, sp.z, sp.w, rr, o, d, hb, disc);
        if (!(disc < T(0))) { if (!(hb > T(0)) || disc > hb * hb) push(i); }
    };

    const int big0 = w.n_groups_pad * GS;
    for (int b = 0; b < w.n_big; ++b) {
        const int i = big0 + b;
        member(V4{gx[4 * i], gx[4 * i + 1], gx[4 * i + 2], gx[4 * i + 3]}, i);
    }

    const V3<T> ocs = {o.x - w.cs[0], o.y - w.cs[1], o.z - w.cs[2]};
    const T s2 = dot(d, d);
    const T eps_p = (s2 > T(1) ? s2 - T(1) : T(0)) + (sizeof(T) == 4 ? T(2.4e-7) : T(4.5e-16)) * s2;
    const T margin = (w.kappa * (s2 > T(1) ? s2 : T(1)) + T(2) * t_sqrt(eps_p)) * ((t_sqrt(dot(ocs, ocs)) + w.rs) + T(1));
    auto safe_inv = [](T x) { const T e = T(1e-9); const T y = (x < e && x > -e) ? (x < T(0) ? -e : e) : x; return T(1) / y; };
    const V3<T> inv = {safe_inv(d.x), safe_inv(d.y), safe_inv(d.z)};
    const V3<T> op = {o.x + margin, o.y + margin, o.z + margin};
    const V3<T> om = {o.x - margin, o.y - margin, o.z - margin};

    struct Box { T lx, ly, lz, l_, hx, hy, hz, h_; };
    cptr gb = (cptr)(uintptr_t)w.box;
    auto ldb = [](cptr p, int k) -> Box { return Box{p[8 * k], p[8 * k + 1], p[8 * k + 2], p[8 * k + 3], p[8 * k + 4], p[8 * k + 5], p[8 * k + 6], p[8 * k + 7]}; };
    Box A[G], B[G];
#pragma unroll
    for (int k = 0; k < G; ++k) A[k] = ldb(gb, k);
    cptr pw = gb;
    auto test1 = [&](const Box &bx, uint32_t &mask) {
        const T x0 = (bx.lx - op.x) * inv.x, x1 = (bx.hx - om.x) * inv.x;
        const T y0 = (bx.ly - op.y) * inv.y, y1 = (bx.hy - om.y) * inv.y;
        const T z0 = (bx.lz - op.z) * inv.z, z1 = (bx.hz - om.z) * inv.z;
        const T tn = t_max(t_max(t_min(x0, x1), t_min(y0, y1)), t_min(z0, z1));
        const T tf = t_min(t_min(t_max(x0, x1), t_max(y0, y1)), t_max(z0, z1));
        const T sgn = tf - t_max(tn, T(0));
        mask = __builtin_amdgcn_alignbit(mask, sign_word(sgn), 31);
    };
    for (int base = 0; base < w.n_groups_pad; base += RTW_SPHERE_WORD) {
        uint32_t mask = 0;
        const int left = w.n_groups_pad - base;
        const int npairs = left >= RTW_SPHERE_WORD ? RTW_SPHERE_WORD / (2 * G) : left / (2 * G);
        for (int q = 0; q < npairs; ++q, pw += 2 * G * 8) {
            test1(A[0], mask);
            __builtin_amdgcn_sched_barrier(0);
#pragma unroll
            for (int k = 0; k < G; ++k) B[k] = ldb(pw, G + k);
            __builtin_amdgcn_sched_barrier(0);
#pragma unroll
            for (int k = 1; k < G; ++k) test1(A[k], mask);
            __builtin_amdgcn_sched_barrier(0);
            test1(B[0], mask);
            __builtin_amdgcn_sched_barrier(0);
#pragma unroll
            for (int k = 0; k < G; ++k) A[k] = ldb(pw, 2 * G + k);
            __builtin_amdgcn_sched_barrier(0);
#pragma unroll
            for (int k = 1; k < G; ++k) test1(B[k], mask);
            __builtin_amdgcn_sched_barrier(0);
        }
        clk.lap(2);
        uint32_t m = ~mask;
        if (left < RTW_SPHERE_WORD) m <<= (RTW_SPHERE_WORD - npairs * 2 * G);
        while (__any(m != 0u)) {
            if (m != 0u) {
                const int b = __clz((int)m);
                m &= ~(0x80000000u >> b);
                const int first = (base + b) * GS;
#pragma unroll 1
                for (int h = 0; h < GS; h += RTW_CULL_L2) {
                    V4 sp[RTW_CULL_L2];
#pragma unroll
                    for (int j = 0; j < RTW_CULL_L2; ++j) sp[j] = src[first + h + j];
#pragma unroll
                    for (int j = 0; j < RTW_CULL_L2; ++j) member(sp[j], first + h + j);
                }
            }
        }
        clk.lap(4);
    }
    resolve_candidates_anyorder<T, STRIDE>(w.numerics, src, w.mat0, orig, o, d, tmin, closest, idx, list, cnt);
    clk.lap(5);
    t_hit = closest;
    return idx;
}

template <typename T>
__device__ __forceinline__ void stage_cull_scene(const CullScene<T> &w, typename Vec4<T>::type *dst, unsigned short *dst_orig) {
    const int n = cull_exact_count(w);
    for (int i = threadIdx.x; i < n; i += blockDim.x) { dst[i] = w.exact[i]; dst_orig[i] = w.orig[i]; }
}

template <typename T>
__device__ __forceinline__ void stage_scene(const DevScene<T> &w, typename Vec4<T>::type *dst) {
    const int n_alloc = scene_geom_alloc(w.n, w.n_pad);
    for (int i = threadIdx.x; i < n_alloc; i += blockDim.x) dst[i] = w.geom[i];
}

}
```

raytracingweekend.jl_amd/csrc/rtw_scan_mfma.hpp:

```cpp
#pragma once
#include "rtw_scan.hpp"
#include "rtw_cull_tables.hpp"
#include "rtw_probes.hpp"

namespace rtw {

#define RTW_PAIR_CAP 512
typedef _Float16 rtw_h8 __attribute__((ext_vector_type(8)));
typedef float rtw_f16v __attribute__((ext_vector_type(16)));

__host__ __device__ inline int cull_tab_words(int blocks) { return ((blocks + 31) / 32 > 0 ? (blocks + 31) / 32 : 1) * RTW_CULL_TAB_WORDS; }
struct CullGrid {
    float inv[3], off[3];
};

struct MfmaCull {
    const uint4 *ops;
    const float *box;
    int blocks;
    float cs[3], rs;
    const void *mat0;
    float glo[3], ghi[3];
    int n_huge;
    int n_exact;
    CullGrid grid;
    const unsigned *tab;
};

struct WaveScratch {
    unsigned *pairs;
    unsigned long long *keys;
    unsigned *kidx;
    unsigned cap = 5 * RTW_PAIR_CAP / 16;
    unsigned cap2 = 3 * RTW_PAIR_CAP / 8;
};

__device__ __forceinline__ unsigned split_f16(float x) {
    unsigned w;
    __asm__("v_cvt_f16_f32_e32 %0, %1\n\tv_fma_mixhi_f16 %0, %1, 1.0, -%0 op_sel_hi:[0,0,1]" : "=&v"(w) : "v"(x));
    return w;
}
__device__ __forceinline__ float lane_get(float v, unsigned src_lane) {
    return __int_as_float(__builtin_amdgcn_ds_bpermute((int)(src_lane << 2), __float_as_int(v)));
}
__device__ __forceinline__ double lane_get(double v, unsigned src_lane) {
    const long long b = __double_as_longlong(v);
    const unsigned lo = (unsigned)__builtin_amdgcn_ds_bpermute((int)(src_lane << 2), (int)(unsigned)b);
    const unsigned hi = (unsigned)__builtin_amdgcn_ds_bpermute((int)(src_lane << 2), (int)(unsigned)((unsigned long long)b >> 32));
    return __longlong_as_double((long long)(((unsigned long long)hi << 32) | lo));
}

#ifndef RTW_INLANE_FILTER
#define RTW_INLANE_FILTER 1
#endif
#ifndef RTW_PRECHECK_GROUPS
#define RTW_PRECHECK_GROUPS 1
#endif
#ifndef RTW_SCAN_SKIP
#define RTW_SCAN_SKIP 1
#endif

struct NoOrig {};
template <typename T, bool WITH_R, typename SRC, typename ORIG = NoOrig, typename SINK = NoSink>
__device__ __forceinline__ void test_singles(int num, SRC src, [[maybe_unused]] const typename Vec4<T>::type *rad, V3<T> o, V3<T> d, T tmin, const WaveScratch &ws, const unsigned *singles, unsigned n, unsigned lane, ORIG orig, unsigned *prof, [[maybe_unused]] SINK sink = SINK()) {
    constexpr bool CULLED = !__is_same(ORIG, NoOrig);
    using V4 = typename Vec4<T>::type;
    for (unsigned p0 = 0; p0 < n; p0 += 64u) {
        const unsigned p = p0 + lane;
        const bool valid = p < n;
        const unsigned e = singles[valid ? p : 0u];
        if (prof) { prof[0] += 1u; prof[1] += (unsigned)__popcll(__ballot(valid)); }
        const unsigned owner = ((e >> 16) & 31u) + ((e & 16u) << 1), sph = (e & 0xffefu) + ((e >> 17) & 16u);
        const V3<T> po = {lane_get(o.x, owner), lane_get(o.y, owner), lane_get(o.z, owner)};
        const V3<T> pd = {lane_get(d.x, owner), lane_get(d.y, owner), lane_get(d.z, owner)};
        const V4 s = src[sph];
        if constexpr (SINK::on()) { if (valid) { if constexpr (CULLED) sink.cand(owner, (int)orig[sph]); else sink.cand(owner, (int)sph); } }
        T hb, disc, root = 0;
        if constexpr (WITH_R) sphere_disc_n<T, NUM_REFERENCE_FMA2>(s.x, s.y, s.z, s.w, rad[sph].x, po, pd, hb, disc);
        else sphere_disc<T>(num, s.x, s.y, s.z, s.w, T(0), po, pd, hb, disc);
        const bool hit = valid && sphere_root<T>(hb, disc, tmin, (T)__builtin_huge_val(), root);
        unsigned tie = sph;
        if constexpr (CULLED) tie = ((unsigned)orig[sph] << 16) | sph;
        if constexpr (sizeof(T) == 4) {
            if (hit) {
                const unsigned low = CULLED ? ((0xffffu - (tie >> 16)) << 16) | (tie & 0xffffu) : 0xffffffffu - tie;
                const unsigned long long key = ((unsigned long long)__float_as_uint(root) << 32) | (unsigned long long)low;
                __hip_atomic_fetch_min(&ws.keys[owner], key, __ATOMIC_RELAXED, __HIP_MEMORY_SCOPE_WORKGROUP);
            }
        } else {
            const unsigned long long tb = (unsigned long long)__double_as_longlong(root);
            unsigned long long old = 0ull;
            if (hit) old = __hip_atomic_fetch_min(&ws.keys[owner], tb, __ATOMIC_RELAXED, __HIP_MEMORY_SCOPE_WORKGROUP);
            __builtin_amdgcn_wave_barrier();
            const unsigned long long cur = ws.keys[owner];
            if (hit && tb == cur && old > tb) ws.kidx[owner] = 0u;
            __builtin_amdgcn_wave_barrier();
            if (hit && tb == cur) __hip_atomic_fetch_max(&ws.kidx[owner], tie + 1u, __ATOMIC_RELAXED, __HIP_MEMORY_SCOPE_WORKGROUP);
            __builtin_amdgcn_wave_barrier();
        }
    }
}
template <typename T, bool WITH_R, typename SRC, typename ORIG = NoOrig, typename SINK = NoSink>
__device__ __forceinline__ void resolve_pairs_impl(int num, SRC src, [[maybe_unused]] const typename Vec4<T>::type *rad, V3<T> o, V3<T> d, T tmin, const WaveScratch &ws, unsigned n, unsigned lane, ORIG orig = ORIG(), unsigned *prof = nullptr, SINK sink = SINK()) {
    __builtin_amdgcn_wave_barrier();
    const uint2 *list = reinterpret_cast<const uint2 *>(ws.pairs);
    unsigned *singles = ws.pairs + 2u * ws.cap;
    unsigned total = 0;
    for (unsigned p0 = 0; p0 < n; p0 += 64u) {
        const unsigned p = p0 + lane;
        const uint2 e = list[p < n ? p : 0u];
        unsigned m = p < n ? e.x : 0u;
        const unsigned code31 = e.y + 31u;
        for (;;) {
            const unsigned long long act = __ballot(m != 0u);
            if (prof) prof[2] += 1u;
            if (!act) break;
            if (total + 64u > ws.cap2) {
                __builtin_amdgcn_wave_barrier();
                test_singles<T, WITH_R>(num, src, rad, o, d, tmin, ws, singles, total, lane, orig, prof, sink);
                __builtin_amdgcn_wave_barrier();
                total = 0;
            }
            if (m != 0u) {
                const unsigned z = (unsigned)__builtin_ctz(m);
                m &= m - 1u;
                singles[__builtin_amdgcn_mbcnt_hi((unsigned)(act >> 32), __builtin_amdgcn_mbcnt_lo((unsigned)act, total))] = code31 - z;
            }
            total += (unsigned)__popcll(act);
        }
    }
    __builtin_amdgcn_wave_barrier();
    test_singles<T, WITH_R>(num, src, rad, o, d, tmin, ws, singles, total, lane, orig, prof, sink);
    __builtin_amdgcn_wave_barrier();
}

template <typename T, typename SRC, typename RAD, typename ORIG = NoOrig, typename SINK = NoSink>
__device__ __forceinline__ void resolve_pairs(int num, SRC src, RAD rad, V3<T> o, V3<T> d, T tmin, const WaveScratch &ws, unsigned n, unsigned lane, ORIG orig = ORIG(), unsigned *prof = nullptr, SINK sink = SINK()) {
    if (num == NUM_REFERENCE_FMA2) resolve_pairs_impl<T, true>(num, src, rad(), o, d, tmin, ws, n, lane, orig, prof, sink);
    else resolve_pairs_impl<T, false>(num, src, nullptr, o, d, tmin, ws, n, lane, orig, prof, sink);
}

template <typename T, typename SRC, typename ORIG = NoOrig, typename CLK = NoClock, typename SINK = NoSink>
__device__ __forceinline__ int hit_world_mfma(const DevScene<T> &w, SRC src, V3<T> o, V3<T> d, bool has_ray, T tmin, T &t_hit,
                                              const WaveScratch &ws, unsigned lane, CLK &&clk = NoClock(),
                                              const MfmaCull *mc = nullptr, ORIG orig = ORIG(), SINK sink = SINK()) {
    constexpr bool CULLED = !__is_same(ORIG, NoOrig);
    auto rad = [&]() -> const typename Vec4<T>::type * { if constexpr (CULLED) return (const typename Vec4<T>::type *)mc->mat0; else return w.mat0; };
    const float ox = (float)o.x, oy = (float)o.y, oz = (float)o.z, dx = (float)d.x, dy = (float)d.y, dz = (float)d.z;
    const float s2 = __builtin_fmaf(dz, dz, __builtin_fmaf(dy, dy, dx * dx));
    const float oinf = __builtin_fmaxf(__builtin_fmaxf(__builtin_fabsf(ox), __builtin_fabsf(oy)), __builtin_fabsf(oz));
    const bool ok = has_ray && s2 <= 1.0009f && oinf <= w.mf_o_max;
    if constexpr (SINK::on()) { if (has_ray) sink.ray(lane, ok, w.mf_sc); }
    const float q = __builtin_fmaf(oz, dz, __builtin_fmaf(oy, dy, ox * dx));
    const float oo = __builtin_fmaf(oz, oz, __builtin_fmaf(oy, oy, ox * ox));
    const float o1 = (__builtin_fabsf(ox) + __builtin_fabsf(oy)) + __builtin_fabsf(oz);
    const float oop = __builtin_fmaf(oo, w.mf_oo_keep, -(w.mf_o1_coef * o1));
    const float tq = w.mf_sigma2 * __builtin_fmaf(q, q, -oop);
    const float z = ok ? 1.0f : 0.0f, z2 = z + z, zs2 = z2 * w.mf_sc;
    const float fp[3] = {__builtin_fmaf(-q, dx, ox) * zs2, __builtin_fmaf(-q, dy, oy) * zs2, __builtin_fmaf(-q, dz, oz) * zs2};
    const float dx2 = dx * z2, dy2 = dy * z2, dz2 = dz * z2;
    const float fq[6] = {dx2 * dx, dy2 * dy, dz2 * dz, (dx2 + dx2) * dy, (dx2 + dx2) * dz, (dy2 + dy2) * dz};
    const float tx = ok ? tq : (has_ray ? 60000.0f * 32768.0f : -60000.0f * 32768.0f);
    const uint4 *ops_base = CULLED ? mc->ops : w.mf_ops;
    auto pa_of = [&](int b) { return ops_base + (size_t)(unsigned)b * 128u; };
    const int n_blocks = CULLED ? mc->blocks : w.mf_blocks;
    [[maybe_unused]] auto block_sets = [&](int base_, unsigned &v0_, unsigned &v1_) {
        float cox = ox, coy = oy, coz = oz, cdx = dx, cdy = dy, cdz = dz, cs2 = s2;
        __asm__ volatile("" : "+v"(cox), "+v"(coy), "+v"(coz), "+v"(cdx), "+v"(cdy), "+v"(cdz), "+v"(cs2));
        unsigned bin_lo[3], bin_hi[3];
        const float ex = cox - mc->cs[0], ey = coy - mc->cs[1], ez = coz - mc->cs[2];
        const float eps_p = (cs2 > 1.0f ? cs2 - 1.0f : 0.0f) + 2.4e-7f * cs2;
        const float m = 1.001f * (0.00390625f * (cs2 > 1.0f ? cs2 : 1.0f) + 2.0f * __builtin_amdgcn_sqrtf(eps_p)) *
                        ((__builtin_amdgcn_sqrtf(__builtin_fmaf(ez, ez, __builtin_fmaf(ey, ey, ex * ex))) + mc->rs) + 1.0f);
        auto safe_inv = [](float x) {
            const float mag = __builtin_fmaxf(__builtin_fabsf(x), 1e-9f);
            return __builtin_amdgcn_rcpf(__uint_as_float((__float_as_uint(mag) & 0x7fffffffu) | (__float_as_uint(x) & 0x80000000u)));
        };
        const float ix = safe_inv(cdx), iy = safe_inv(cdy), iz = safe_inv(cdz);
        const float x0 = ((mc->glo[0] - m) - cox) * ix, x1 = ((mc->ghi[0] + m) - cox) * ix;
        const float y0 = ((mc->glo[1] - m) - coy) * iy, y1 = ((mc->ghi[1] + m) - coy) * iy;
        const float z0 = ((mc->glo[2] - m) - coz) * iz, z1 = ((mc->ghi[2] + m) - coz) * iz;
        const float tn = __builtin_fmaxf(__builtin_fmaxf(__builtin_fmaxf(__builtin_fminf(x0, x1), __builtin_fminf(y0, y1)), __builtin_fminf(z0, z1)), 0.0f);
        const float tf = __builtin_fminf(__builtin_fminf(__builtin_fmaxf(x0, x1), __builtin_fmaxf(y0, y1)), __builtin_fmaxf(z0, z1));
        const float m2 = m + m;
        const float ax = __builtin_fmaf(tn, cdx, cox), ay = __builtin_fmaf(tn, cdy, coy), az = __builtin_fmaf(tn, cdz, coz);
        const float bx = __builtin_fmaf(tf, cdx, cox), by = __builtin_fmaf(tf, cdy, coy), bz = __builtin_fmaf(tf, cdz, coz);
        const bool hits_class = tf >= tn;
        const float lo3[3] = {__builtin_fminf(ax, bx) - m2, __builtin_fminf(ay, by) - m2, __builtin_fminf(az, bz) - m2};
        const float hi3[3] = {__builtin_fmaxf(ax, bx) + m2, __builtin_fmaxf(ay, by) + m2, __builtin_fmaxf(az, bz) + m2};
        const CullGrid &G = mc->grid;
        auto binf = [](float u) {
            const unsigned b = (unsigned)__builtin_amdgcn_fmed3f(u, 0.0f, (float)RTW_CULL_BINS - 0.5f);
            __builtin_assume(b < (unsigned)RTW_CULL_BINS);
            return b;
        };
#pragma unroll
        for (int k = 0; k < 3; ++k) {
            bin_lo[k] = binf(__builtin_fmaf(lo3[k], G.inv[k], G.off[k]));
            bin_hi[k] = binf(__builtin_fmaf(hi3[k], G.inv[k], G.off[k]));
        }
        const bool cells_ok = ok && hits_class;
        const unsigned flag_word = 6u * RTW_CULL_BINS + (has_ray ? (ok ? 0u : 1u) : 2u);
        const unsigned *t = mc->tab + (base_ >> 5) * RTW_CULL_TAB_WORDS;
        unsigned mine = (t[0 * RTW_CULL_BINS + bin_hi[0]] & t[1 * RTW_CULL_BINS + bin_lo[0]]) & (t[2 * RTW_CULL_BINS + bin_hi[1]] & t[3 * RTW_CULL_BINS + bin_lo[1]]) &
                        (t[4 * RTW_CULL_BINS + bin_hi[2]] & t[5 * RTW_CULL_BINS + bin_lo[2]]);
        mine = (cells_ok ? mine : 0u) | t[flag_word];
        mine |= (unsigned)__builtin_amdgcn_update_dpp(0, (int)mine, 0xB1, 0xf, 0xf, true);
        mine |= (unsigned)__builtin_amdgcn_update_dpp(0, (int)mine, 0x4E, 0xf, 0xf, true);
        mine |= (unsigned)__builtin_amdgcn_update_dpp(0, (int)mine, 0x141, 0xf, 0xf, true);
        mine |= (unsigned)__builtin_amdgcn_update_dpp(0, (int)mine, 0x140, 0xf, 0xf, true);
        v0_ = (unsigned)__builtin_amdgcn_readlane((int)mine, 0) | (unsigned)__builtin_amdgcn_readlane((int)mine, 16);
        v1_ = (unsigned)__builtin_amdgcn_readlane((int)mine, 32) | (unsigned)__builtin_amdgcn_readlane((int)mine, 48);
    };
    uint4 A1 = {0u, 0u, 0u, 0u}, A2 = {0u, 0u, 0u, 0u};
    if constexpr (!CULLED) { A1 = pa_of(0)[lane]; A2 = pa_of(0)[lane + 64u]; }
    unsigned sq[6], sp[3];
#pragma unroll
    for (int k = 0; k < 6; ++k) sq[k] = split_f16(fq[k]);
#pragma unroll
    for (int k = 0; k < 3; ++k) sp[k] = split_f16(fp[k]);
    const _Float16 t1 = (_Float16)(tx * (1.0f / 32768.0f));
    const float trem = tx - 32768.0f * (float)t1;
    const unsigned x23 = split_f16(trem * (1.0f / 16.0f));
    const unsigned sb = ok ? 0x7800u : 0u, ss = ok ? 0x4c00u : 0u;
    auto dup = [](unsigned v) { return __builtin_amdgcn_perm(v, v, 0x01000100u); };
    auto cat = [](unsigned a, unsigned b) { return __builtin_amdgcn_alignbit(b, a, 16); };
    const unsigned g0[8] = {dup(sq[0]), cat(sq[0], sq[1]), sq[1], dup(sq[2]),
                            sq[5], dup(sp[0]), cat(sp[0], sp[1]), sp[1]};
    const unsigned g1[8] = {cat(sq[2], sq[3]), sq[3], dup(sq[4]), cat(sq[4], sq[5]),
                            dup(sp[2]), cat(sp[2], sb), ss | ((unsigned)__builtin_bit_cast(unsigned short, t1) << 16), x23};
    unsigned h0[8], h1[8];
#pragma unroll
    for (int k = 0; k < 8; ++k) {
        const auto sw = __builtin_amdgcn_permlane32_swap(g0[k], g1[k], false, false);
        h0[k] = sw[0]; h1[k] = sw[1];
    }
    RTW_PROBE_OPERANDS_TWICE();
    rtw_h8 B1[2], B2[2];
    {
        const uint4 q10 = {h0[0], h0[1], h0[2], h0[3]}, q11 = {h1[0], h1[1], h1[2], h1[3]};
        const uint4 q20 = {h0[4], h0[5], h0[6], h0[7]}, q21 = {h1[4], h1[5], h1[6], h1[7]};
        B1[0] = __builtin_bit_cast(rtw_h8, q10); B1[1] = __builtin_bit_cast(rtw_h8, q11);
        B2[0] = __builtin_bit_cast(rtw_h8, q20); B2[1] = __builtin_bit_cast(rtw_h8, q21);
    }
    const unsigned lane_const = lane << 16;
    unsigned total = 0;
    {
        unsigned long long key0 = ~0ull;
        [[maybe_unused]] unsigned kidx0 = 0u;
        using V4 = typename Vec4<T>::type;
        const int n_huge = CULLED ? (RTW_INLANE_FILTER ? mc->n_exact : mc->n_huge) : w.n_huge;
        for (int hgi = 0; hgi < n_huge; ++hgi) {
            int si;
            if constexpr (CULLED) si = __builtin_amdgcn_readfirstlane((int)mc->tab[6 * RTW_CULL_BINS + 4 + hgi]);
            else si = hgi == 0 ? w.huge[0] : w.huge[1];
            const V4 sg = src[si];
            if constexpr (SINK::on()) { if (has_ray) { if constexpr (CULLED) sink.inlane(lane, (int)orig[si]); else sink.inlane(lane, si); } }
            T hb_, disc_, root_ = 0;
            T rr_ = T(0);
            if (w.numerics == NUM_REFERENCE_FMA2) rr_ = rad()[si].x;
            sphere_disc<T>(w.numerics, sg.x, sg.y, sg.z, sg.w, rr_, o, d, hb_, disc_);
            if (has_ray && sphere_root<T>(hb_, disc_, tmin, (T)__builtin_huge_val(), root_)) {
                unsigned tie = (unsigned)si;
                if constexpr (CULLED) tie = ((unsigned)orig[si] << 16) | (unsigned)si;
                if constexpr (sizeof(T) == 4) {
                    const unsigned low = CULLED ? ((0xffffu - (tie >> 16)) << 16) | (tie & 0xffffu) : 0xffffffffu - tie;
                    const unsigned long long k = ((unsigned long long)__float_as_uint((float)root_) << 32) | (unsigned long long)low;
                    key0 = k < key0 ? k : key0;
                } else {
                    const unsigned long long tb = (unsigned long long)__double_as_longlong((double)root_);
                    if (tb < key0 || (tb == key0 && tie + 1u > kidx0)) { key0 = tb; kidx0 = tie + 1u; }
                }
            }
        }
        if constexpr (sizeof(T) == 4) ws.keys[lane] = key0;
        else { ws.keys[lane] = key0; ws.kidx[lane] = kidx0; }
    }
    if constexpr (CULLED && RTW_INLANE_FILTER) {
        using V4 = typename Vec4<T>::type;
        for (int hgi = mc->n_exact; hgi < mc->n_huge; ++hgi) {
            const int si = __builtin_amdgcn_readfirstlane((int)mc->tab[6 * RTW_CULL_BINS + 4 + hgi]);
            const V4 sg = src[si];
            if constexpr (SINK::on()) { if (has_ray) sink.inlane(lane, (int)orig[si]); }
            T hb_, disc_;
            T rr_ = T(0);
            if (w.numerics == NUM_REFERENCE_FMA2) rr_ = rad()[si].x;
            sphere_disc<T>(w.numerics, sg.x, sg.y, sg.z, sg.w, rr_, o, d, hb_, disc_);
            const bool cand = has_ray && !(disc_ < T(0));
            const unsigned long long cm = __ballot(cand);
            if (cm) {
                if (total + 64u > ws.cap) { resolve_pairs<T>(w.numerics, src, rad, o, d, tmin, ws, total, lane, orig, nullptr, sink); total = 0; }
                if (cand) {
                    const unsigned b = ((lane >> 5) << 4) | ((unsigned)si & 15u);
                    const unsigned code = ((((unsigned)si >> 4) & 1u) << 21) | ((lane & 31u) << 16) | (((unsigned)si >> 5) << 5);
                    const unsigned pos = __builtin_amdgcn_mbcnt_hi((unsigned)(cm >> 32), __builtin_amdgcn_mbcnt_lo((unsigned)cm, total));
                    reinterpret_cast<uint2 *>(ws.pairs)[pos] = uint2{0x80000000u >> b, code};
                }
                total += (unsigned)__popcll(cm);
            }
        }
    }
    constexpr bool use_prio = RTW_SCAN_PRIO != 0;
    if (use_prio) __builtin_amdgcn_s_setprio(sizeof(T) == 4 ? 0 : 1);
    for (int base = 0; base < n_blocks; base += CULLED ? 32 : n_blocks) {
    [[maybe_unused]] unsigned vote0 = 0, vote1 = 0, todo = 0;
    int blk = base;
    if constexpr (CULLED) {
        block_sets(base, vote0, vote1);
        todo = vote0 | vote1;
        clk.count(7, (unsigned)(n_blocks - base < 32 ? n_blocks - base : 32));
        clk.count(6, (unsigned)((n_blocks - base < 32 ? n_blocks - base : 32) - __popc(todo)));
        if (!todo) continue;
        blk = base + (int)__builtin_ctz(todo);
        todo &= todo - 1u;
        A1 = pa_of(blk)[lane]; A2 = pa_of(blk)[lane + 64u];
    }
    for (bool more = true; more;) {
        const int cur = blk;
        [[maybe_unused]] bool do_half0 = true, do_half1 = true;
        if constexpr (CULLED) {
            do_half0 = ((vote0 >> (cur - base)) & 1u) != 0u;
            do_half1 = ((vote1 >> (cur - base)) & 1u) != 0u;
            more = todo != 0u;
            blk = more ? base + (int)__builtin_ctz(todo) : cur + 1;
            todo &= todo - 1u;
        } else {
            blk = cur + 1;
            more = blk < n_blocks;
        }
        unsigned mask = 0;
        bool any_cand = false;
        const rtw_f16v zero = {0, 0, 0, 0, 0, 0, 0, 0, 0, 0, 0, 0, 0, 0, 0, 0};
        auto collect = [&](rtw_f16v &Wv) {
            constexpr int NG = RTW_PRECHECK_GROUPS, GS = 16 / NG;
#pragma unroll
            for (int g = 0; g < NG; ++g) {
                const int r0 = g * GS;
                unsigned t = __builtin_amdgcn_bitop3_b32(__float_as_uint(Wv[r0]), __float_as_uint(Wv[r0 + 1]), __float_as_uint(Wv[r0 + 2]), 0x80);
#pragma unroll
                for (int r = r0 + 3; r < r0 + GS - 1; r += 2) t = __builtin_amdgcn_bitop3_b32(t, __float_as_uint(Wv[r]), __float_as_uint(Wv[r + 1]), 0x80);
                t &= __float_as_uint(Wv[r0 + GS - 1]);
                if (RTW_SCAN_SKIP && !__any((int)t >= 0)) {
                    mask = (mask << GS) | ((1u << GS) - 1u);
                } else {
                    if (RTW_SCAN_SKIP) __asm__ volatile("" : "+v"(Wv));
#pragma unroll
                    for (int r = r0; r < r0 + GS; ++r) mask = __builtin_amdgcn_alignbit(mask, __float_as_uint(Wv[r]), 31);
                    any_cand = true;
                    clk.count(26, 1u);
                }
            }
        };
        [[maybe_unused]] auto eval = [&](const rtw_f16v &Wv) {
#pragma unroll
            for (int r = 0; r < 16; ++r) mask = __builtin_amdgcn_alignbit(mask, __float_as_uint(Wv[r]), 31);
        };
        auto filter_pair = [&](const uint4 &a1, const uint4 &a2, const rtw_h8 &b1, const rtw_h8 &b2) -> rtw_f16v {
            RTW_PROBE_FILTER_PAIR_REPLACED(a1, a2, b1, b2);
            rtw_f16v Wp = __builtin_amdgcn_mfma_f32_32x32x16_f16(__builtin_bit_cast(rtw_h8, a1), b1, zero, 0, 0, 0);
            Wp = __builtin_amdgcn_mfma_f32_32x32x16_f16(__builtin_bit_cast(rtw_h8, a2), b2, Wp, 0, 0, 0);
            RTW_PROBE_FILTER_PAIR_AGAIN(Wp, a1, a2, b1, b2);
            return Wp;
        };
        constexpr unsigned HB = 16u;
        {
            if (!CULLED || do_half0) {
                rtw_f16v Wv = filter_pair(A1, A2, B1[0], B2[0]);
                RTW_PROBE_EVAL_TWICE(Wv);
                collect(Wv);
            } else {
                mask = (1u << HB) - 1u;
            }
        }
        {
            if (!CULLED || do_half1) {
                rtw_f16v Wv = filter_pair(A1, A2, B1[1], B2[1]);
                __builtin_amdgcn_sched_barrier(0);
                A1 = pa_of(blk)[lane]; A2 = pa_of(blk)[lane + 64u];
                __builtin_amdgcn_sched_barrier(0);
                RTW_PROBE_EVAL_TWICE(Wv);
                collect(Wv);
            } else {
                A1 = pa_of(blk)[lane]; A2 = pa_of(blk)[lane + 64u];
                mask = (mask << HB) | ((1u << HB) - 1u);
            }
        }
        clk.lap(2);
        if (RTW_SCAN_SKIP && !any_cand) {
            if constexpr (!CULLED) { clk.count(7, 1u); clk.count(6, 1u); }
            continue;
        }
        unsigned m = ~mask;
        if constexpr (!CULLED) {
            clk.count(7, 1u);
            if (!__any(m != 0u)) clk.count(6, 1u);
        }
        const unsigned long long act = __ballot(m != 0u);
        clk.count(27, 1u);
        if (total + 64u > ws.cap) {
            clk.lap(4);
            { unsigned pr[3] = {0u, 0u, 0u}; resolve_pairs<T>(w.numerics, src, rad, o, d, tmin, ws, total, lane, orig, clk.on() ? pr : nullptr, sink); clk.count(13, total); clk.count(14, pr[0]); clk.count(15, pr[1]); clk.count(28, pr[2]); }
            total = 0;
            clk.lap(5);
        }
        RTW_PROBE_EXTRACT_TWICE();
        if (m != 0u) {
            const unsigned pos = __builtin_amdgcn_mbcnt_hi((unsigned)(act >> 32), __builtin_amdgcn_mbcnt_lo((unsigned)act, total));
            reinterpret_cast<uint2 *>(ws.pairs)[pos] = uint2{m, lane_const + (unsigned)cur * 32u};
        }
        total += (unsigned)__popcll(act);
        clk.lap(4);
    }
    }
    if (use_prio) __builtin_amdgcn_s_setprio(sizeof(T) == 4 ? 1 : 0);
    { unsigned pr[3] = {0u, 0u, 0u}; resolve_pairs<T>(w.numerics, src, rad, o, d, tmin, ws, total, lane, orig, clk.on() ? pr : nullptr, sink); clk.count(13, total); clk.count(14, pr[0]); clk.count(15, pr[1]); clk.count(28, pr[2]); }
    RTW_PROBE_RESOLVE_TWICE();
    clk.lap(5);
    int idx;
    if constexpr (sizeof(T) == 4) {
        const unsigned long long k = ws.keys[lane];
        idx = k == ~0ull ? -1 : (CULLED ? (int)((unsigned)k & 0xffffu) : (int)(0xffffffffu - (unsigned)k));
        t_hit = __uint_as_float((unsigned)(k >> 32));
    } else {
        const unsigned long long k = ws.keys[lane];
        const unsigned ki = ws.kidx[lane];
        idx = ki == 0u ? -1 : (CULLED ? (int)((ki - 1u) & 0xffffu) : (int)ki - 1);
        t_hit = __longlong_as_double((long long)k);
    }
    if (!has_ray) idx = -1;
    return idx;
}

}
```

raytracingweekend.jl_amd/csrc/rtw_units.hpp:

```cpp
#pragma once
#include "rtw_device.hpp"

namespace rtw {

enum UnitOp {
    U_HIT_SPHERE = 0, U_REFLECT = 1, U_REFRACT = 2, U_REFLECTANCE = 3, U_SCATTER = 4,
    U_GET_RAY = 5, U_SKYCOLOR = 6, U_RNG = 7, U_HIT_WORLD = 8, U_RAY_COLOR = 9,
    U_HIT_WORLD_LDS = 10,
    U_HIT_WORLD_CULL = 11,
    U_FX_SUM = 12,
    U_HIT_WORLD_MFMA = 13,
    U_HIT_WORLD_MFMA_CULL = 14,
    U_NEAR_ZERO = 15,
    U_EXACT_MATH = 16,
    U_SINK_LDS = 17, U_SINK_CULL = 18, U_SINK_MFMA = 19, U_SINK_MFMA_CULL = 20,
    U_NUM_OPS = 21
};
__host__ __device__ inline bool unit_is_sink(int op) { return op >= U_SINK_LDS && op <= U_SINK_MFMA_CULL; }
#define RTW_SINK_SPHERES 512
#define RTW_SINK_SLOTS 18

__host__ __device__ inline int unit_in_slots(int op) {
    switch (op) {
        case U_HIT_SPHERE: return 12;
        case U_REFLECT: return 6;
        case U_REFRACT: return 7;
        case U_REFLECTANCE: return 2;
        case U_SCATTER: return 18;
        case U_GET_RAY: return 4;
        case U_SKYCOLOR: return 3;
        case U_RNG: return 2;
        case U_NEAR_ZERO: return 3;
        case U_EXACT_MATH: return 2;
        case U_HIT_WORLD: case U_HIT_WORLD_LDS: case U_HIT_WORLD_CULL: case U_HIT_WORLD_MFMA: case U_HIT_WORLD_MFMA_CULL: return 8;
        case U_SINK_LDS: case U_SINK_CULL: case U_SINK_MFMA: case U_SINK_MFMA_CULL: return 8;
        case U_RAY_COLOR: return 9;
        case U_FX_SUM: return 8;
    }
    return 0;
}
__host__ __device__ inline int unit_out_slots(int op) {
    switch (op) {
        case U_HIT_SPHERE: return 9;
        case U_REFLECT: return 3;
        case U_REFRACT: return 3;
        case U_REFLECTANCE: return 1;
        case U_SCATTER: return 11;
        case U_GET_RAY: return 8;
        case U_SKYCOLOR: return 3;
        case U_RNG: return 6;
        case U_NEAR_ZERO: return 2;
        case U_EXACT_MATH: return 4;
        case U_HIT_WORLD: case U_HIT_WORLD_LDS: case U_HIT_WORLD_CULL: case U_HIT_WORLD_MFMA: case U_HIT_WORLD_MFMA_CULL: return 9;
        case U_SINK_LDS: case U_SINK_CULL: case U_SINK_MFMA: case U_SINK_MFMA_CULL: return RTW_SINK_SLOTS;
        case U_RAY_COLOR: return 6;
        case U_FX_SUM: return 2;
    }
    return 0;
}

template <typename T>
__device__ __forceinline__ V3<T> ld3(const double *p) { return {(T)p[0], (T)p[1], (T)p[2]}; }
template <typename T>
__device__ __forceinline__ void st3(double *p, V3<T> v) { p[0] = (double)v.x; p[1] = (double)v.y; p[2] = (double)v.z; }
__device__ __forceinline__ uint64_t as_u64(double d) { return (uint64_t)__double_as_longlong(d); }
__device__ __forceinline__ double as_f64(uint64_t u) { return __longlong_as_double((long long)u); }

struct CandSink {
    double *rows;
    unsigned n_live;
    unsigned self;
    static constexpr bool on() { return true; }
    __device__ void ray(unsigned lane, bool ok, float sc) {
        if (lane < n_live) { rows[lane * RTW_SINK_SLOTS] = ok ? 1.0 : 0.0; rows[lane * RTW_SINK_SLOTS + 1] = (double)sc; }
    }
    __device__ void bit(unsigned lane, int slot0, int i) {
        if (lane < n_live && (unsigned)i < (unsigned)RTW_SINK_SPHERES)
            atomicOr(reinterpret_cast<unsigned long long *>(rows + lane * RTW_SINK_SLOTS + slot0 + (i >> 6)), 1ull << (i & 63));
    }
    __device__ void cand(unsigned lane, int i) { bit(lane, 2, i); }
    __device__ void inlane(unsigned lane, int i) { bit(lane, 10, i); }
};

template <typename T>
__global__ void unit_kernel(int op, int count, const double *__restrict__ in, double *__restrict__ out,
                            DevScene<T> scene, CullScene<T> cull, Camera<T> cam) {
    using V4 = typename Vec4<T>::type;
    const int gid = blockIdx.x * blockDim.x + threadIdx.x;
    __shared__ unsigned short s_list[RTW_LIST_CAP * 64];
    extern __shared__ __attribute__((aligned(16))) unsigned char u_smem[];
    unsigned short *my_list = s_list + threadIdx.x;
    const bool live = gid < count;
    const double *x = in + (size_t)gid * unit_in_slots(op);
    double *y = out + (size_t)gid * unit_out_slots(op);
    const bool coop = op == U_HIT_WORLD || op == U_RAY_COLOR || op == U_HIT_WORLD_LDS || op == U_HIT_WORLD_CULL || op == U_HIT_WORLD_MFMA || op == U_HIT_WORLD_MFMA_CULL || unit_is_sink(op);
    const int wave0 = gid - (int)(threadIdx.x & 63u);
    const CandSink sink = {out + (size_t)wave0 * RTW_SINK_SLOTS, (unsigned)(count - wave0 < 64 ? count - wave0 : 64), threadIdx.x & 63u};
    if (!coop && !live) return;
    switch (op) {
        case U_HIT_SPHERE: {
            V3<T> c = ld3<T>(x), o = ld3<T>(x + 4), d = ld3<T>(x + 7);
            T r = (T)x[3], tmin = (T)x[10], tmax = (T)x[11];
            T hb, disc, root;
            sphere_disc<T>(scene.numerics, c.x, c.y, c.z, r * r, r, o, d, hb, disc);
            for (int k = 0; k < 9; ++k) y[k] = 0.0;
            if (sphere_root<T>(hb, disc, tmin, tmax, root)) {
                HitRec<T> rec;
                make_hitrec<T>(c, r, o, d, root, rec);
                y[0] = 1.0; y[1] = (double)rec.t; st3(y + 2, rec.p); st3(y + 5, rec.n); y[8] = rec.front ? 1.0 : 0.0;
            }
        } break;
        case U_REFLECT: st3(y, reflect(ld3<T>(x), ld3<T>(x + 3))); break;
        case U_REFRACT: st3(y, refract(ld3<T>(x), ld3<T>(x + 3), (T)x[6])); break;
        case U_REFLECTANCE: y[0] = (double)reflectance((T)x[0], (T)x[1]); break;
        case U_SCATTER: {
            Rng rng = {as_u64(x[0]), as_u64(x[1])};
            HitRec<T> rec;
            rec.t = (T)x[10]; rec.p = ld3<T>(x + 11); rec.n = ld3<T>(x + 14); rec.front = x[17] != 0.0;
            V3<T> nd, att;
            scatter<T>(rng, (int)x[2], ld3<T>(x + 3), (T)x[6], ld3<T>(x + 7), rec, nd, att);
            y[0] = as_f64(rng.x); y[1] = as_f64(rng.y);
            st3(y + 2, rec.p); st3(y + 5, nd); st3(y + 8, att);
        } break;
        case U_GET_RAY: {
            Rng rng = {as_u64(x[0]), as_u64(x[1])};
            V3<T> o, d;
            get_ray(rng, cam, (T)x[2], (T)x[3], o, d);
            y[0] = as_f64(rng.x); y[1] = as_f64(rng.y);
            st3(y + 2, o); st3(y + 5, d);
        } break;
        case U_SKYCOLOR: {
            C3 c = skycolor(ld3<T>(x));
            y[0] = c.r; y[1] = c.g; y[2] = c.b;
        } break;
        case U_RNG: {
            Rng rng = {as_u64(x[0]), as_u64(x[1])};
            for (int k = 0; k < 4; ++k) { T u; trand(rng, u); y[2 + k] = (double)u; }
            y[0] = as_f64(rng.x); y[1] = as_f64(rng.y);
        } break;
        case U_EXACT_MATH: {
            double bad_s = 0, bad_r = 0, first_s = -1, first_r = -1;
            if constexpr (sizeof(T) == 4) {
                const unsigned p0 = (unsigned)x[0], n = (unsigned)x[1];
                for (unsigned k = 0; k < n; ++k) {
                    const unsigned u = p0 + k;
                    const float v = __uint_as_float(u);
                    const unsigned a = __float_as_uint(t_sqrt(v)), b = __float_as_uint(__builtin_sqrtf(v));
                    const unsigned c = __float_as_uint(t_rcp(v)), e = __float_as_uint(1.0f / v);
                    const bool nan_ab = (a & 0x7fffffffu) > 0x7f800000u && (b & 0x7fffffffu) > 0x7f800000u;
                    const bool nan_ce = (c & 0x7fffffffu) > 0x7f800000u && (e & 0x7fffffffu) > 0x7f800000u;
                    if (a != b && !nan_ab) { bad_s += 1; if (first_s < 0) first_s = (double)u; }
                    if (c != e && !nan_ce) { bad_r += 1; if (first_r < 0) first_r = (double)u; }
                }
            }
            y[0] = bad_s; y[1] = bad_r; y[2] = first_s; y[3] = first_r;
        } break;
        case U_NEAR_ZERO: {
            const V3<T> v = ld3<T>(x);
            y[0] = near_zero(v) ? 1.0 : 0.0;
            y[1] = (double)dot(v, v);
        } break;
        case U_HIT_WORLD: {
            V3<T> o = {0, 0, 0}, d = {0, 0, 1};
            T tmn = 0, tmx = 0;
            if (live) { o = ld3<T>(x); d = ld3<T>(x + 3); tmn = (T)x[6]; tmx = (T)x[7]; }
            T t_hit;
            int idx = hit_world<T, 64>(scene, scene.geom, o, d, tmn, tmx, t_hit, my_list);
            if (!live) return;
            for (int k = 0; k < 9; ++k) y[k] = 0.0;
            y[0] = (double)idx;
            if (idx >= 0) {
                auto g = scene.geom[idx];
                auto m0 = scene.mat0[idx];
                HitRec<T> rec;
                make_hitrec<T>({g.x, g.y, g.z}, m0.x, o, d, t_hit, rec);
                y[1] = (double)rec.t; st3(y + 2, rec.p); st3(y + 5, rec.n); y[8] = rec.front ? 1.0 : 0.0;
            }
        } break;
        case U_HIT_WORLD_LDS: case U_HIT_WORLD_CULL: {
            V4 *lds_geom = reinterpret_cast<V4 *>(u_smem);
            unsigned short *lds_orig = reinterpret_cast<unsigned short *>(lds_geom + (op == U_HIT_WORLD_CULL ? cull_exact_count(cull) : 0));
            if (op == U_HIT_WORLD_CULL) stage_cull_scene<T>(cull, lds_geom, lds_orig); else stage_scene<T>(scene, lds_geom);
            __syncthreads();
            V3<T> o = {0, 0, 0}, d = {0, 0, 1};
            T tmn = 0, tmx = 0;
            if (live) { o = ld3<T>(x); d = ld3<T>(x + 3); tmn = (T)x[6]; tmx = (T)x[7]; }
            T t_hit;
            int idx;
            if (op == U_HIT_WORLD_CULL)
                idx = hit_world_cull<T, 64>(cull, (const V4 *)lds_geom, (const unsigned short *)lds_orig, o, d, tmn, tmx, t_hit, my_list);
            else
                idx = hit_world<T, 64>(scene, (const V4 *)lds_geom, o, d, tmn, tmx, t_hit, my_list);
            if (!live) return;
            for (int k = 0; k < 9; ++k) y[k] = 0.0;
            y[0] = (double)(idx >= 0 && op == U_HIT_WORLD_CULL ? (int)cull.orig[idx] : idx);
            if (idx >= 0) {
                const V4 g = op == U_HIT_WORLD_CULL ? cull.exact[idx] : scene.geom[idx];
                const V4 m0 = op == U_HIT_WORLD_CULL ? cull.mat0[idx] : scene.mat0[idx];
                HitRec<T> rec;
                make_hitrec<T>({g.x, g.y, g.z}, m0.x, o, d, t_hit, rec);
                y[1] = (double)rec.t; st3(y + 2, rec.p); st3(y + 5, rec.n); y[8] = rec.front ? 1.0 : 0.0;
            }
        } break;
        case U_HIT_WORLD_MFMA: {
            __shared__ __attribute__((aligned(8))) unsigned s_pairs[RTW_PAIR_CAP];
            __shared__ unsigned long long s_keys[64];
            __shared__ unsigned s_kidx[64];
            V4 *lds_geom = reinterpret_cast<V4 *>(u_smem);
            stage_scene<T>(scene, lds_geom);
            __syncthreads();
            V3<T> o = {0, 0, 0}, d = {0, 0, 1};
            if (live) { o = ld3<T>(x); d = ld3<T>(x + 3); }
            const T tmn = (T)in[6];
            T t_hit;
            const WaveScratch ws = {s_pairs, s_keys, s_kidx};
            int idx = -1;
            if (scene.mf_ops) idx = hit_world_mfma<T>(scene, (const V4 *)lds_geom, o, d, live, tmn, t_hit, ws, threadIdx.x & 63u);
            if (!live) return;
            for (int k = 0; k < 9; ++k) y[k] = 0.0;
            y[0] = (double)idx;
            if (idx >= 0) {
                const V4 g = scene.geom[idx];
                const V4 m0 = scene.mat0[idx];
                HitRec<T> rec;
                make_hitrec<T>({g.x, g.y, g.z}, m0.x, o, d, t_hit, rec);
                y[1] = (double)rec.t; st3(y + 2, rec.p); st3(y + 5, rec.n); y[8] = rec.front ? 1.0 : 0.0;
            }
        } break;
        case U_HIT_WORLD_MFMA_CULL: {
            __shared__ __attribute__((aligned(8))) unsigned c_pairs[RTW_PAIR_CAP];
            __shared__ unsigned long long c_keys[64];
            __shared__ unsigned c_kidx[64];
            V4 *lds_geom = reinterpret_cast<V4 *>(u_smem);
            unsigned short *lds_orig = reinterpret_cast<unsigned short *>(lds_geom + cull_exact_count(cull));
            stage_cull_scene<T>(cull, lds_geom, lds_orig);
            __syncthreads();
            V3<T> o = {0, 0, 0}, d = {0, 0, 1};
            if (live) { o = ld3<T>(x); d = ld3<T>(x + 3); }
            const T tmn = (T)in[6];
            T t_hit;
            const WaveScratch ws = {c_pairs, c_keys, c_kidx};
            const MfmaCull mc = mfma_cull_of(cull);
            int idx = -1;
            if (cull.mf_ops) idx = hit_world_mfma<T>(scene, (const V4 *)lds_geom, o, d, live, tmn, t_hit, ws, threadIdx.x & 63u, NoClock(), &mc, (const unsigned short *)lds_orig);
            if (!live) return;
            for (int k = 0; k < 9; ++k) y[k] = 0.0;
            y[0] = (double)(idx >= 0 ? (int)cull.orig[idx] : idx);
            if (idx >= 0) {
                const V4 g = cull.exact[idx];
                const V4 m0 = cull.mat0[idx];
                HitRec<T> rec;
                make_hitrec<T>({g.x, g.y, g.z}, m0.x, o, d, t_hit, rec);
                y[1] = (double)rec.t; st3(y + 2, rec.p); st3(y + 5, rec.n); y[8] = rec.front ? 1.0 : 0.0;
            }
        } break;
        case U_SINK_LDS: case U_SINK_CULL: {
            V4 *lds_geom = reinterpret_cast<V4 *>(u_smem);
            unsigned short *lds_orig = reinterpret_cast<unsigned short *>(lds_geom + (op == U_SINK_CULL ? cull_exact_count(cull) : 0));
            if (op == U_SINK_CULL) stage_cull_scene<T>(cull, lds_geom, lds_orig); else stage_scene<T>(scene, lds_geom);
            __syncthreads();
            V3<T> o = {0, 0, 0}, d = {0, 0, 1};
            T tmn = 0, tmx = 0;
            if (live) { o = ld3<T>(x); d = ld3<T>(x + 3); tmn = (T)x[6]; tmx = (T)x[7]; }
            T t_hit;
            if (op == U_SINK_CULL)
                hit_world_cull<T, 64>(cull, (const V4 *)lds_geom, (const unsigned short *)lds_orig, o, d, tmn, tmx, t_hit, my_list, NoClock(), sink);
            else
                hit_world<T, 64>(scene, (const V4 *)lds_geom, o, d, tmn, tmx, t_hit, my_list, NoClock(), sink);
        } break;
        case U_SINK_MFMA: case U_SINK_MFMA_CULL: {
            __shared__ __attribute__((aligned(8))) unsigned k_pairs[RTW_PAIR_CAP];
            __shared__ unsigned long long k_keys[64];
            __shared__ unsigned k_kidx[64];
            V4 *lds_geom = reinterpret_cast<V4 *>(u_smem);
            unsigned short *lds_orig = reinterpret_cast<unsigned short *>(lds_geom + (op == U_SINK_MFMA_CULL ? cull_exact_count(cull) : 0));
            if (op == U_SINK_MFMA_CULL) stage_cull_scene<T>(cull, lds_geom, lds_orig); else stage_scene<T>(scene, lds_geom);
            __syncthreads();
            V3<T> o = {0, 0, 0}, d = {0, 0, 1};
            if (live) { o = ld3<T>(x); d = ld3<T>(x + 3); }
            const T tmn = (T)in[6];
            T t_hit;
            const WaveScratch ws = {k_pairs, k_keys, k_kidx};
            if (op == U_SINK_MFMA_CULL) {
                const MfmaCull mc = mfma_cull_of(cull);
                hit_world_mfma<T>(scene, (const V4 *)lds_geom, o, d, live, tmn, t_hit, ws, threadIdx.x & 63u, NoClock(), &mc, (const unsigned short *)lds_orig, sink);
            } else {
                hit_world_mfma<T>(scene, (const V4 *)lds_geom, o, d, live, tmn, t_hit, ws, threadIdx.x & 63u, NoClock(), nullptr, NoOrig(), sink);
            }
        } break;
        case U_FX_SUM: {
            unsigned long long lo = 0, hi = 0, bad = 0;
            for (int k = 0; k < 8; ++k) {
                unsigned long long l, h;
                if (fx_from_double(x[k], l, h)) { const unsigned long long old = lo; lo += l; hi += h + (lo < old ? 1ull : 0ull); }
                else bad += 1;
            }
            y[0] = bad ? __builtin_nan("") : fx_to_double(lo, hi);
            y[1] = (double)bad;
        } break;
        case U_RAY_COLOR: {
            Rng rng = {1, 2};
            V3<T> o = {0, 0, 0}, d = {0, 0, 1};
            int depth = 0;
            if (live) { rng = {as_u64(x[0]), as_u64(x[1])}; o = ld3<T>(x + 2); d = ld3<T>(x + 5); depth = (int)x[8]; }
            double tr = 1, tg = 1, tb = 1, cr = 0, cg = 0, cb = 0;
            unsigned segs = 0;
            bool active = depth > 0;
            while (__any(active)) {
                T t_hit;
                int idx = hit_world<T, 64>(scene, scene.geom, o, d, (T)1e-4, (T)__builtin_huge_val(), t_hit, my_list);
                if (!active) continue;
                segs++;
                if (idx < 0) {
                    C3 sky = skycolor(d);
                    cr = tr * sky.r; cg = tg * sky.g; cb = tb * sky.b;
                    active = false;
                    continue;
                }
                auto g = scene.geom[idx];
                auto m0 = scene.mat0[idx];
                auto m1 = scene.mat1[idx];
                HitRec<T> rec;
                make_hitrec<T>({g.x, g.y, g.z}, m0.x, o, d, t_hit, rec);
                V3<T> nd, att;
                scatter<T>(rng, (int)m0.z, {m1.x, m1.y, m1.z}, m0.y, d, rec, nd, att);
                tr = tr * (double)att.x; tg = tg * (double)att.y; tb = tb * (double)att.z;
                o = rec.p; d = nd;
                depth -= 1;
                if (depth <= 0) active = false;
            }
            if (!live) return;
            y[0] = as_f64(rng.x); y[1] = as_f64(rng.y);
            y[2] = cr; y[3] = cg; y[4] = cb; y[5] = (double)segs;
        } break;
    }
}

}
```

Baseline: 5668.

## Hoist reciprocals for jitter and normal divisions, plus misc wave-vote and load tweaks

Replaces the per-component IEEE divisions in the hit-record normal with one refined reciprocal and three FMA-corrected quotients, guarded by a wave-uniform range check that falls back to true division. Precomputes refined reciprocals of width and height in LDS for the jitter divisions. Also switches __any/__all to raw 64-bit ballots, loads hit geometry through explicit global address-space pointers taken from an LDS table, and counts samples once per chunk via an LDS atomic instead of a per-iteration ballot. These aim to cut division and vote overhead in the hot path, at the cost of extra guard logic and LDS traffic, and add a unit test that checks the division shortcut for bit-exactness.

```diff
diff --git a/raytracingweekend.jl_amd/csrc/rtw_div.hpp b/raytracingweekend.jl_amd/csrc/rtw_div.hpp
--- /dev/null
+++ b/raytracingweekend.jl_amd/csrc/rtw_div.hpp
@@ -0,0 +1,33 @@
+#pragma once
+
+#if defined(__HIPCC__) || defined(__CUDACC__)
+#define RTW_DIV_HD __host__ __device__ __forceinline__
+#else
+#define RTW_DIV_HD inline
+#endif
+
+namespace rtw {
+
+#define RTW_DIV_LO 0x1p-60f
+#define RTW_DIV_HI 0x1p60f
+
+RTW_DIV_HD float div_refine_rcp(float b, float y0) {
+    const float e = __builtin_fmaf(-b, y0, 1.0f);
+    return __builtin_fmaf(e, y0, y0);
+}
+RTW_DIV_HD float div_quotient(float a, float b, float y) {
+    float q = a * y;
+    float e = __builtin_fmaf(-b, q, a);
+    q = __builtin_fmaf(e, y, q);
+    e = __builtin_fmaf(-b, q, a);
+    return __builtin_fmaf(e, y, q);
+}
+RTW_DIV_HD bool div_significand_ok(float b) { return (__builtin_bit_cast(unsigned, b) & 0x007fffffu) != 0x007fffffu; }
+RTW_DIV_HD bool div_in_guard(float a, float b) {
+    const float fa = __builtin_fabsf(a), fb = __builtin_fabsf(b);
+    return fa >= RTW_DIV_LO && fa <= RTW_DIV_HI && fb >= RTW_DIV_LO && fb <= RTW_DIV_HI && div_significand_ok(b);
+}
+RTW_DIV_HD bool div_jitter_denominator_ok(float b) { return b >= 1.0f && b <= 0x1p31f; }
+RTW_DIV_HD float div_jitter_prep(float b) { return div_refine_rcp(b, 1.0f / b); }
+
+}
diff --git a/raytracingweekend.jl_amd/csrc/rtw_kernels.hpp b/raytracingweekend.jl_amd/csrc/rtw_kernels.hpp
--- a/raytracingweekend.jl_amd/csrc/rtw_kernels.hpp
+++ b/raytracingweekend.jl_amd/csrc/rtw_kernels.hpp
@@ -80,6 +80,8 @@
     JobCache jobs;
     Camera<T> cam;
     KParams P;
+    alignas(16) const typename Vec4<T>::type *hit_tab[4];
+    alignas(16) T jit[4];
 };
 
 template <bool ON> struct PhaseClock {
@@ -326,6 +328,12 @@
     if (lane == 0) S->job = g;
 }
 
+template <typename T> __device__ __forceinline__ typename Vec4<T>::type load_global_v4(const typename Vec4<T>::type *p) {
+    typedef T Raw4 __attribute__((ext_vector_type(4)));
+    const Raw4 v = *(const Raw4 __attribute__((address_space(1))) *)p;
+    return {v.x, v.y, v.z, v.w};
+}
+
 template <typename T, bool PROFILE, bool LDS_SCENE, bool CULL, bool MFMA = false, int NUMK = -1, bool BATCH = false, bool ACCUM = false>
 __global__ __launch_bounds__(256, (TraceWavesOf<T, CULL, MFMA>::value)) void trace_kernel(KParams P_arg, Camera<T> cam_arg, DevScene<T> scene,
                                                    CullScene<T> cull, T *__restrict__ out, DevCounters *ctr, BatchArgs<T> batch, AccumArgs accum) {
@@ -355,7 +363,15 @@
     unsigned short *lds_orig = reinterpret_cast<unsigned short *>(lds_geom + (CULL ? cull_exact_count(cull) : 0));
     [[maybe_unused]] unsigned *lds_tab = reinterpret_cast<unsigned *>(reinterpret_cast<unsigned char *>(lds_orig) + (CULL ? ((size_t)cull_exact_count(cull) * sizeof(unsigned short) + 15) / 16 * 16 : 0));
     if (threadIdx.x < P_arg.n_slots) { JobSlot *S0 = sh->slot(threadIdx.x, P_arg.slot_stride); S0->ready_seq = RTW_SLOT_FREE; S0->job = 0u; }
-    if (threadIdx.x == 0) { sh->ticket = 0u; sh->eof = 0u; sh->fin_waves = 0u; sh->fin_segments = 0ull; sh->fin_samples = 0ull; sh->jobs.jc = 0ull; sh->jobs.jc_lock = 0u; sh->jobs.queue_off = 0u; sh->jobs.last_g = 0u; sh->jobs.static_used = 0u; sh->cam = cam_arg; sh->P = P_arg; }
+    if (threadIdx.x == 0) { sh->ticket = 0u; sh->eof = 0u; sh->fin_waves = 0u; sh->fin_segments = 0ull; sh->fin_samples = 0ull; sh->jobs.jc = 0ull; sh->jobs.jc_lock = 0u; sh->jobs.queue_off = 0u; sh->jobs.last_g = 0u; sh->jobs.static_used = 0u; sh->cam = cam_arg; sh->P = P_arg;
+                            sh->hit_tab[0] = CULL ? cull.exact : scene.geom; sh->hit_tab[1] = CULL ? cull.mat0 : scene.mat0; sh->hit_tab[2] = CULL ? cull.mat1 : scene.mat1; sh->hit_tab[3] = nullptr; }
+    constexpr bool jit_short = sizeof(T) == 4 && RTW_EXACT_FAST_MATH != 0 && !RTW_PROBE_FASTDIV_ON;
+    if constexpr (jit_short) {
+        if (threadIdx.x == 0) {
+            const float wf = (float)P_arg.width, hf = (float)P_arg.height;
+            sh->jit[0] = wf; sh->jit[1] = div_jitter_prep(wf); sh->jit[2] = hf; sh->jit[3] = div_jitter_prep(hf);
+        }
+    }
     const KParams &P = sh->P;
     if (LDS_SCENE) {
         if (CULL) stage_cull_scene<T>(cull, lds_geom, lds_orig);
@@ -373,7 +389,8 @@
     bool have_ticket = false;
     unsigned tk_seq = 0, tk_b = 0;
 
-    unsigned long long n_segments = 0, n_samples = 0;
+    unsigned long long n_segments = 0;
+    [[maybe_unused]] unsigned long long n_samples = 0;
 
     bool alive = true;
     bool have_item = false;
@@ -384,8 +401,8 @@
     Rng rng = {1, 2};
     V3<T> ro = {0, 0, 0}, rd = {0, 0, 1};
     double thr_r = 1, thr_g = 1, thr_b = 1;
-    const T w_div = (T)(float)P.width;
-    const T h_div = (T)(float)P.height;
+    [[maybe_unused]] const T w_div = (T)(float)P.width;
+    [[maybe_unused]] const T h_div = (T)(float)P.height;
 
     PhaseClock<PROFILE> clk;
     for (;;) {
@@ -393,14 +410,14 @@
         T t_hit = 0;
         int idx = -1;
         if constexpr (MFMA && CULL) {
-            if (__any(has_ray)) {
+            if (wave_any(has_ray)) {
                 MfmaCull mc = mfma_cull_of(cull);
                 if (LDS_SCENE) mc.tab = lds_tab;
                 if (LDS_SCENE) idx = hit_world_mfma<T>(scene, (const V4 *)lds_geom, ro, rd, has_ray, (T)1e-4, t_hit, ws, lane, clk, &mc, (const unsigned short *)lds_orig);
                 else idx = hit_world_mfma<T>(scene, cull.exact, ro, rd, has_ray, (T)1e-4, t_hit, ws, lane, clk, &mc, cull.orig);
             }
         } else if constexpr (MFMA) {
-            if (__any(has_ray)) {
+            if (wave_any(has_ray)) {
                 if (LDS_SCENE) idx = hit_world_mfma<T>(scene, (const V4 *)lds_geom, ro, rd, has_ray, (T)1e-4, t_hit, ws, lane, clk);
                 else idx = hit_world_mfma<T>(scene, scene.geom, ro, rd, has_ray, (T)1e-4, t_hit, ws, lane, clk);
             }
@@ -417,7 +434,7 @@
         }
         n_segments += (unsigned long long)__popcll(__ballot(has_ray));
         clk.lap(2);
-        if (PROFILE) { clk.count(8, 1u); clk.count(9, (unsigned)__popcll(__ballot(has_ray))); if (!__any(has_ray)) clk.count(10, 1u); }
+        if (PROFILE) { clk.count(8, 1u); clk.count(9, (unsigned)__popcll(__ballot(has_ray))); if (!wave_any(has_ray)) clk.count(10, 1u); }
 
         const bool hit = has_ray && idx >= 0;
         if constexpr (MFMA) {
@@ -568,6 +585,7 @@
                         int s0 = (int)chunk * P.chunk_spp;
                         if constexpr (ACCUM) s0 = (int)(chunk + (unsigned)accum.chunk_begin) * P.chunk_spp;
                         samples_left = min(P.spp, s0 + P.chunk_spp) - s0;
+                        if constexpr (!PROFILE) __hip_atomic_fetch_add(&sh->fin_samples, (unsigned long long)samples_left, __ATOMIC_RELAXED, __HIP_MEMORY_SCOPE_WORKGROUP);
                         jitter = s0 != 0;
                         ref_depth = pool_slot * 16u + px;
                         have_item = true;
@@ -580,18 +598,21 @@
             }
             if (PROFILE) clk.count(12, (unsigned)__popcll(__ballot(need && alive && !have_item)));
         }
-        if (!__any(alive)) break;
+        if (!wave_any(alive)) break;
         clk.lap(0);
 
         int todo = PATH_READY;
         V3<T> vec = {0, 0, 0};
         T vscale_ = 1;
         int kind = 0;
-        if (PROFILE && __any(hit)) clk.count(23, 1u);
+        if (PROFILE && wave_any(hit)) clk.count(23, 1u);
         if (hit) {
-            const V4 g = CULL ? cull.exact[idx] : scene.geom[idx];
-            const V4 m0 = CULL ? cull.mat0[idx] : scene.mat0[idx];
-            const V4 m1 = CULL ? cull.mat1[idx] : scene.mat1[idx];
+            const V4 *const tab_g = PROFILE ? (CULL ? cull.exact : scene.geom) : sh->hit_tab[0];
+            const V4 *const tab_m0 = PROFILE ? (CULL ? cull.mat0 : scene.mat0) : sh->hit_tab[1];
+            const V4 *const tab_m1 = PROFILE ? (CULL ? cull.mat1 : scene.mat1) : sh->hit_tab[2];
+            const V4 g = load_global_v4<T>(tab_g + idx);
+            const V4 m0 = load_global_v4<T>(tab_m0 + idx);
+            const V4 m1 = load_global_v4<T>(tab_m1 + idx);
             HitRec<T> rec;
             make_hitrec<T>({g.x, g.y, g.z}, m0.x, ro, rd, t_hit, rec);
             kind = (int)m0.z;
@@ -611,8 +632,16 @@
             T du = 0, dv = 0;
             if (jitter) {
                 T r1, r2;
-                trand(rng, r1); du = RTW_DIV(r1, w_div);
-                trand(rng, r2); dv = RTW_DIV(r2, h_div);
+                trand(rng, r1);
+                trand(rng, r2);
+                if constexpr (jit_short) {
+                    const float4 jd = *reinterpret_cast<const float4 *>(sh->jit);
+                    du = div_quotient(r1, jd.x, jd.y);
+                    dv = div_quotient(r2, jd.z, jd.w);
+                } else {
+                    du = RTW_DIV(r1, w_div);
+                    dv = RTW_DIV(r2, h_div);
+                }
             }
             const JobSlot *S = sh->slot((ref_depth & RTW_REF_MASK) >> 4, P.slot_stride);
             const unsigned px = ref_depth & 15u;
@@ -623,8 +652,8 @@
             jitter = true;
             samples_left -= 1;
         }
-        n_samples += (unsigned long long)__popcll(__ballot(new_sample));
-        if (PROFILE && __any(new_sample)) clk.count(24, 1u);
+        if constexpr (PROFILE) n_samples += (unsigned long long)__popcll(__ballot(new_sample));
+        if (PROFILE && wave_any(new_sample)) clk.count(24, 1u);
 
         const bool ball = todo == PATH_BALL;
         V3<T> rp = {0, 0, 0};
@@ -642,10 +671,10 @@
             if (pending) len2 = T(1);
 #else
             if constexpr (PROFILE) {
-                if (__any(pending)) clk.count(17, 1u);
-                while (__any(pending)) {
+                if (wave_any(pending)) clk.count(17, 1u);
+                while (wave_any(pending)) {
                     clk.count(16, 1u);
-                    if (__any(ball && pending)) clk.count(29, 1u);
+                    if (wave_any(ball && pending)) clk.count(29, 1u);
                     if (pending) { len2 = reject_trial<T>(rng, ball, rp); pending = !(len2 <= T(1)); }
                 }
             }
@@ -666,18 +695,20 @@
                 const Camera<T> cam = batch.cams[sh->slot((ref_depth & RTW_REF_MASK) >> 4, P.slot_stride)->pad];
                 camera_ray_raw<T>(cam, su, sv, rp.x, rp.y, ro, vec);
             } else {
-                const Camera<T> cam = sh->cam;
+                unsigned cam_off = (unsigned)(reinterpret_cast<const unsigned char *>(&sh->cam) - smem);
+                __asm__ volatile("" : "+v"(cam_off));
+                const Camera<T> cam = *reinterpret_cast<const Camera<T> *>(smem + cam_off);
                 camera_ray_raw<T>(cam, su, sv, rp.x, rp.y, ro, vec);
             }
             todo = PATH_NORM;
             thr_r = thr_g = thr_b = 1.0;
             ref_depth = (ref_depth & RTW_REF_MASK) | ((unsigned)P.max_depth << RTW_REF_BITS);
         }
-        if (PROFILE && __any(todo == PATH_NORM)) clk.count(25, 1u);
+        if (PROFILE && wave_any(todo == PATH_NORM)) clk.count(25, 1u);
         if (todo == PATH_NORM) rd = normalize(vec);
         if (ball || new_sample || todo == PATH_NORM) has_ray = ref_depth > RTW_REF_MASK;
         clk.lap(1);
-        if (!__any(has_ray)) __builtin_amdgcn_s_sleep(2);
+        if (!wave_any(has_ray)) __builtin_amdgcn_s_sleep(2);
     }
 
     if (PROFILE && lane == 0) {
@@ -685,7 +716,7 @@
     }
     if (lane == 0) {
         __hip_atomic_fetch_add(&sh->fin_segments, n_segments, __ATOMIC_RELAXED, __HIP_MEMORY_SCOPE_WORKGROUP);
-        __hip_atomic_fetch_add(&sh->fin_samples, n_samples, __ATOMIC_RELAXED, __HIP_MEMORY_SCOPE_WORKGROUP);
+        if constexpr (PROFILE) __hip_atomic_fetch_add(&sh->fin_samples, n_samples, __ATOMIC_RELAXED, __HIP_MEMORY_SCOPE_WORKGROUP);
         if ((threadIdx.x >> 6) < 4u) __hip_atomic_store(&sh->t_wave[4u + (threadIdx.x >> 6)], wall_clock64(), __ATOMIC_RELAXED, __HIP_MEMORY_SCOPE_WORKGROUP);
         const unsigned nw = blockDim.x >> 6;
         if (__hip_atomic_fetch_add(&sh->fin_waves, 1u, __ATOMIC_ACQ_REL, __HIP_MEMORY_SCOPE_WORKGROUP) == nw - 1u) {
diff --git a/raytracingweekend.jl_amd/csrc/rtw_path.hpp b/raytracingweekend.jl_amd/csrc/rtw_path.hpp
--- a/raytracingweekend.jl_amd/csrc/rtw_path.hpp
+++ b/raytracingweekend.jl_amd/csrc/rtw_path.hpp
@@ -1,6 +1,7 @@
 #pragma once
 #include <hip/hip_runtime.h>
 #include <stdint.h>
+#include "rtw_div.hpp"
 
 namespace rtw {
 
@@ -14,12 +15,18 @@
 template <> struct Vec4<float> { using type = float4; };
 template <> struct Vec4<double> { using type = double4; };
 
+__device__ __forceinline__ bool wave_any(bool p) { return __builtin_amdgcn_ballot_w64(p) != 0ull; }
+template <typename... B> __device__ __forceinline__ bool wave_all(bool p, B... more) {
+    return (__builtin_amdgcn_ballot_w64(p) & ... & __builtin_amdgcn_ballot_w64(more)) == __builtin_amdgcn_ballot_w64(true);
+}
+
 #ifndef RTW_EXACT_FAST_MATH
 #define RTW_EXACT_FAST_MATH 1
 #endif
 __device__ __forceinline__ float t_sqrt(float x) {
 #if RTW_EXACT_FAST_MATH
-    if (__all(x >= 0x1p-100f && x <= 0x1p100f)) {
+    __asm__("" : "+v"(x));
+    if (wave_all(x >= 0x1p-100f, x <= 0x1p100f)) {
         const float y = __builtin_amdgcn_rsqf(x);
         float g = x * y, h = 0.5f * y;
         const float r = __builtin_fmaf(-h, g, 0.5f);
@@ -33,7 +40,7 @@
 __device__ __forceinline__ double t_sqrt(double x) { return __builtin_sqrt(x); }
 __device__ __forceinline__ float t_rcp(float x) {
 #if RTW_EXACT_FAST_MATH
-    if (__all(__builtin_fabsf(x) >= 0x1p-100f && __builtin_fabsf(x) <= 0x1p100f)) {
+    if (wave_all(__builtin_fabsf(x) >= 0x1p-100f, __builtin_fabsf(x) <= 0x1p100f)) {
         float y = __builtin_amdgcn_rcpf(x);
         float e = __builtin_fmaf(-x, y, 1.0f);
         y = __builtin_fmaf(e, y, y);
@@ -44,6 +51,27 @@
     return 1.0f / x;
 }
 __device__ __forceinline__ double t_rcp(double x) { return 1.0 / x; }
+__device__ __forceinline__ float t_div_prep(float b) { return div_refine_rcp(b, __builtin_amdgcn_rcpf(b)); }
+__device__ __forceinline__ float t_div(float a, float b, float y) {
+#if RTW_EXACT_FAST_MATH
+    const float fa = __builtin_fabsf(a), fb = __builtin_fabsf(b);
+    if (wave_all(fa >= RTW_DIV_LO, fa <= RTW_DIV_HI, fb >= RTW_DIV_LO, fb <= RTW_DIV_HI, div_significand_ok(b))) return div_quotient(a, b, y);
+#endif
+    return a / b;
+}
+__device__ __forceinline__ void t_div3(float ax, float ay, float az, float b, float &qx, float &qy, float &qz) {
+#if RTW_EXACT_FAST_MATH
+    const float fx = __builtin_fabsf(ax), fy = __builtin_fabsf(ay), fz = __builtin_fabsf(az), fb = __builtin_fabsf(b);
+    const float hi = __builtin_fmaxf(__builtin_fmaxf(fx, fy), fz), lo = __builtin_fminf(__builtin_fminf(fx, fy), fz);
+    if (wave_all(lo >= RTW_DIV_LO, hi <= RTW_DIV_HI, fb >= RTW_DIV_LO, fb <= RTW_DIV_HI, div_significand_ok(b))) {
+        const float y = t_div_prep(b);
+        qx = div_quotient(ax, b, y); qy = div_quotient(ay, b, y); qz = div_quotient(az, b, y);
+        return;
+    }
+#endif
+    qx = ax / b; qy = ay / b; qz = az / b;
+}
+__device__ __forceinline__ void t_div3(double ax, double ay, double az, double b, double &qx, double &qy, double &qz) { qx = ax / b; qy = ay / b; qz = az / b; }
 __device__ __forceinline__ float t_fma(float a, float b, float c) { return __builtin_fmaf(a, b, c); }
 __device__ __forceinline__ double t_fma(double a, double b, double c) { return __builtin_fma(a, b, c); }
 
@@ -175,7 +203,8 @@
     rec.t = t;
     rec.p = vadd(o, vscale(t, d));
     V3<T> pc = vsub(rec.p, c);
-    V3<T> n_out = {RTW_DIV(pc.x, r), RTW_DIV(pc.y, r), RTW_DIV(pc.z, r)};
+    V3<T> n_out;
+    RTW_DIV3(pc, r, n_out);
     rec.front = dot(d, n_out) < T(0);
     rec.n = rec.front ? n_out : vneg(n_out);
 }
diff --git a/raytracingweekend.jl_amd/csrc/rtw_probes.hpp b/raytracingweekend.jl_amd/csrc/rtw_probes.hpp
--- a/raytracingweekend.jl_amd/csrc/rtw_probes.hpp
+++ b/raytracingweekend.jl_amd/csrc/rtw_probes.hpp
@@ -100,9 +100,13 @@
 #endif
 
 #ifdef RTW_PROBE_FASTDIV
+#define RTW_PROBE_FASTDIV_ON 1
 #define RTW_DIV(a, b) ((a) * ::rtw::probe_rcp(b))
+#define RTW_DIV3(a, b, q) { (q).x = RTW_DIV((a).x, b); (q).y = RTW_DIV((a).y, b); (q).z = RTW_DIV((a).z, b); }
 #define RTW_RSQRT(x) ::rtw::probe_rsq(x)
 #else
+#define RTW_PROBE_FASTDIV_ON 0
 #define RTW_DIV(a, b) ((a) / (b))
+#define RTW_DIV3(a, b, q) t_div3((a).x, (a).y, (a).z, b, (q).x, (q).y, (q).z)
 #define RTW_RSQRT(x) t_rcp(t_sqrt(x))
 #endif
diff --git a/raytracingweekend.jl_amd/csrc/rtw_scan.hpp b/raytracingweekend.jl_amd/csrc/rtw_scan.hpp
--- a/raytracingweekend.jl_amd/csrc/rtw_scan.hpp
+++ b/raytracingweekend.jl_amd/csrc/rtw_scan.hpp
@@ -62,13 +62,13 @@
     };
     int ia = cnt > 0 ? (int)list[0] : 0;
     V4 sa = src[ia];
-    for (int c = 0; __any(c < cnt); c += 2) {
+    for (int c = 0; wave_any(c < cnt); c += 2) {
         const int ib = (c + 1 < cnt) ? (int)list[(c + 1) * STRIDE] : 0;
         const V4 sb = src[ib];
         test(c, ia, sa);
         ia = (c + 2 < cnt) ? (int)list[(c + 2) * STRIDE] : 0;
         sa = src[ia];
-        if (__any(c + 1 < cnt)) test(c + 1, ib, sb);
+        if (wave_any(c + 1 < cnt)) test(c + 1, ib, sb);
     }
 }
 template <typename T, int STRIDE, typename SRC>
@@ -174,12 +174,12 @@
             cnt += 1;
             m &= ~(0x80000000u >> b);
         };
-        if (!__any(m != 0u)) {
-        } else if (!__any(cnt + (int)__popc(m) > RTW_LIST_CAP)) {
-            do { if (m != 0u) push_first(); } while (__any(m != 0u));
+        if (!wave_any(m != 0u)) {
+        } else if (!wave_any(cnt + (int)__popc(m) > RTW_LIST_CAP)) {
+            do { if (m != 0u) push_first(); } while (wave_any(m != 0u));
         } else {
-            while (__any(m != 0u)) {
-                if (__any(cnt >= RTW_LIST_CAP)) {
+            while (wave_any(m != 0u)) {
+                if (wave_any(cnt >= RTW_LIST_CAP)) {
                     clk.lap(4);
                     resolve_candidates<T, STRIDE>(w.numerics, src, w.mat0, o, d, tmin, closest, idx, list, cnt);
                     cnt = 0;
diff --git a/raytracingweekend.jl_amd/csrc/rtw_scan_cull.hpp b/raytracingweekend.jl_amd/csrc/rtw_scan_cull.hpp
--- a/raytracingweekend.jl_amd/csrc/rtw_scan_cull.hpp
+++ b/raytracingweekend.jl_amd/csrc/rtw_scan_cull.hpp
@@ -45,7 +45,7 @@
     using V4 = typename Vec4<T>::type;
     int i_next = cnt > 0 ? (int)list[0] : 0;
     V4 s_next = src[i_next];
-    for (int c = 0; __any(c < cnt); ++c) {
+    for (int c = 0; wave_any(c < cnt); ++c) {
         const int i = i_next;
         const V4 s = s_next;
         i_next = (c + 1 < cnt) ? (int)list[(c + 1) * STRIDE] : 0;
@@ -148,7 +148,7 @@
         clk.lap(2);
         uint32_t m = ~mask;
         if (left < RTW_SPHERE_WORD) m <<= (RTW_SPHERE_WORD - npairs * 2 * G);
-        while (__any(m != 0u)) {
+        while (wave_any(m != 0u)) {
             if (m != 0u) {
                 const int b = __clz((int)m);
                 m &= ~(0x80000000u >> b);
diff --git a/raytracingweekend.jl_amd/csrc/rtw_scan_mfma.hpp b/raytracingweekend.jl_amd/csrc/rtw_scan_mfma.hpp
--- a/raytracingweekend.jl_amd/csrc/rtw_scan_mfma.hpp
+++ b/raytracingweekend.jl_amd/csrc/rtw_scan_mfma.hpp
@@ -340,7 +340,7 @@
 #pragma unroll
                 for (int r = r0 + 3; r < r0 + GS - 1; r += 2) t = __builtin_amdgcn_bitop3_b32(t, __float_as_uint(Wv[r]), __float_as_uint(Wv[r + 1]), 0x80);
                 t &= __float_as_uint(Wv[r0 + GS - 1]);
-                if (RTW_SCAN_SKIP && !__any((int)t >= 0)) {
+                if (RTW_SCAN_SKIP && !wave_any((int)t >= 0)) {
                     mask = (mask << GS) | ((1u << GS) - 1u);
                 } else {
                     if (RTW_SCAN_SKIP) __asm__ volatile("" : "+v"(Wv));
@@ -393,7 +393,7 @@
         unsigned m = ~mask;
         if constexpr (!CULLED) {
             clk.count(7, 1u);
-            if (!__any(m != 0u)) clk.count(6, 1u);
+            if (!wave_any(m != 0u)) clk.count(6, 1u);
         }
         const unsigned long long act = __ballot(m != 0u);
         clk.count(27, 1u);
diff --git a/raytracingweekend.jl_amd/csrc/rtw_units.hpp b/raytracingweekend.jl_amd/csrc/rtw_units.hpp
--- a/raytracingweekend.jl_amd/csrc/rtw_units.hpp
+++ b/raytracingweekend.jl_amd/csrc/rtw_units.hpp
@@ -14,7 +14,8 @@
     U_NEAR_ZERO = 15,
     U_EXACT_MATH = 16,
     U_SINK_LDS = 17, U_SINK_CULL = 18, U_SINK_MFMA = 19, U_SINK_MFMA_CULL = 20,
-    U_NUM_OPS = 21
+    U_DIV_HOIST = 21,
+    U_NUM_OPS = 22
 };
 __host__ __device__ inline bool unit_is_sink(int op) { return op >= U_SINK_LDS && op <= U_SINK_MFMA_CULL; }
 #define RTW_SINK_SPHERES 512
@@ -32,6 +33,7 @@
         case U_RNG: return 2;
         case U_NEAR_ZERO: return 3;
         case U_EXACT_MATH: return 2;
+        case U_DIV_HOIST: return 4;
         case U_HIT_WORLD: case U_HIT_WORLD_LDS: case U_HIT_WORLD_CULL: case U_HIT_WORLD_MFMA: case U_HIT_WORLD_MFMA_CULL: return 8;
         case U_SINK_LDS: case U_SINK_CULL: case U_SINK_MFMA: case U_SINK_MFMA_CULL: return 8;
         case U_RAY_COLOR: return 9;
@@ -51,6 +53,7 @@
         case U_RNG: return 6;
         case U_NEAR_ZERO: return 2;
         case U_EXACT_MATH: return 4;
+        case U_DIV_HOIST: return 4;
         case U_HIT_WORLD: case U_HIT_WORLD_LDS: case U_HIT_WORLD_CULL: case U_HIT_WORLD_MFMA: case U_HIT_WORLD_MFMA_CULL: return 9;
         case U_SINK_LDS: case U_SINK_CULL: case U_SINK_MFMA: case U_SINK_MFMA_CULL: return RTW_SINK_SLOTS;
         case U_RAY_COLOR: return 6;
@@ -155,6 +158,34 @@
             }
             y[0] = bad_s; y[1] = bad_r; y[2] = first_s; y[3] = first_r;
         } break;
+        case U_DIV_HOIST: {
+            double bad_d = 0, bad_3 = 0, bad_j = 0, first = -1;
+            if constexpr (sizeof(T) == 4) {
+                const unsigned a0 = (unsigned)x[0], n = (unsigned)x[1], mode = (unsigned)x[3];
+                const float b = __uint_as_float((unsigned)x[2]);
+                const float yb = mode == 1u ? div_jitter_prep(b) : t_div_prep(b);
+                const auto differ = [](float p, float q) {
+                    const unsigned pu = __float_as_uint(p), qu = __float_as_uint(q);
+                    return pu != qu && !((pu & 0x7fffffffu) > 0x7f800000u && (qu & 0x7fffffffu) > 0x7f800000u);
+                };
+                for (unsigned k = 0; k < n; ++k) {
+                    const unsigned u = a0 + k;
+                    bool bad = false;
+                    if (mode == 1u) {
+                        const float a = __uint_as_float((u & 0x007fffffu) | 0x3f800000u) - 1.0f;
+                        if (differ(div_quotient(a, b, yb), a / b)) { bad_j += 1; bad = true; }
+                    } else {
+                        const float a = __uint_as_float(u), a2 = -a, a3 = a * 3.0f;
+                        if (differ(t_div(a, b, yb), a / b)) { bad_d += 1; bad = true; }
+                        float q1, q2, q3;
+                        t_div3(a, a2, a3, b, q1, q2, q3);
+                        if (differ(q1, a / b) || differ(q2, a2 / b) || differ(q3, a3 / b)) { bad_3 += 1; bad = true; }
+                    }
+                    if (bad && first < 0) first = (double)u;
+                }
+            }
+            y[0] = bad_d; y[1] = bad_3; y[2] = bad_j; y[3] = first;
+        } break;
         case U_NEAR_ZERO: {
             const V3<T> v = ld3<T>(x);
             y[0] = near_zero(v) ? 1.0 : 0.0;
```

After: 5715 (median of 6 runs). No clear change (+0.8%).
